# yuguangnudt/VEC_VAD

Hardware: AMD Instinct MI355X
Metric: spatio-temporal cubes/sec (train step) (higher is better)
Workload: dtype f32

## Files before the change

include/vecvad_hip.h:

```cpp
#ifndef VECVAD_HIP_H
#define VECVAD_HIP_H

#include <stddef.h>
#include <stdint.h>

#ifdef __cplusplus
extern "C" {
#endif

typedef void* vv_stream;

enum vv_status {
  VV_OK = 0,
  VV_ERR_BAD_ARG = 1,
  VV_ERR_LAUNCH = 2,
  VV_ERR_UNSUPPORTED = 3
};

enum vv_in_mode {
  VV_IN_PLAIN = 0,
  VV_IN_ACT = 1,
  VV_IN_POOL = 2,
  VV_IN_CAT = 3,
  VV_IN_CUBE = 4
};

enum vv_conv_kind {
  VV_CONV3 = 0,
  VV_CONVT_FWD = 1,
  VV_CONVT_DGRAD = 2
};

typedef struct vv_view {
  float* ptr;
  int64_t gstride;
  int32_t cstride;
  int32_t coff;
} vv_view;

#define VV_CONV_BF16 1
#define VV_CONV_SRC_BF16 2
#define VV_CONV_OUT_BF16 8
#define VV_CONV_ALLSRC_BF16 16
#define VV_CONV_RELU 32
#define VV_CONV_NO_GEMM16 64
#define VV_CONV_NO_RING 128
typedef struct vv_conv_params {
  int32_t kind;
  int32_t in_mode;
  int32_t G, B;
  int32_t H, W;
  int32_t Cin;
  int32_t CinP;
  int32_t Cout;
  vv_view src0;
  const float* a;
  const float* b;
  int64_t ab_gstride;
  vv_view src1;
  int32_t csplit;
  int32_t pad0;
  const int32_t* chmap;
  const float* w;
  int64_t w_gstride;
  const float* bias;
  int64_t bias_gstride;
  vv_view out;
  float* stats;
  const float* bn_z; int64_t bn_z_gstride;
  const float* bn_a; const float* bn_b; const float* bn_mean; const float* bn_invstd; int64_t bn_gstride;
  float* bn_partial;
  vv_view out1;
  int32_t osplit;
  int32_t pad1;
} vv_conv_params;

int vv_conv_mfma(const vv_conv_params* p, vv_stream stream);
int vv_conv_ntiles(int32_t B, int32_t H, int32_t W);
int vv_convt_dgrad_ntiles(int32_t B, int32_t H, int32_t W, int32_t flags);
int vv_conv_ntiles2(int32_t B, int32_t H, int32_t W, int32_t kind, int32_t flags);

typedef struct vv_wgrad_params {
  int32_t kind;
  int32_t in_mode;
  int32_t G, B, H, W;
  int32_t Cin, CinP, Cout;
  int32_t ksplit;
  vv_view src0; const float* a; const float* b; int64_t ab_gstride;
  vv_view src1; int32_t csplit;
  int32_t pad0;
  const int32_t* chmap;
  vv_view dy;
  float* partial;
  int64_t partial_gstride;
} vv_wgrad_params;

int vv_wgrad_mfma(const vv_wgrad_params* p, vv_stream stream);
int vv_wgrad_ntiles(int32_t kind, int32_t B, int32_t H, int32_t W);

#define VV_WGRAD_X_BF16 2
#define VV_WGRAD_DY_BF16 1
int vv_wgrad_bf16(const vv_wgrad_params* p, vv_stream stream);
int vv_wgrad_bf16_plan(int32_t kind, int32_t B, int32_t H, int32_t W, int32_t CinP, int32_t Cout, int32_t* ntiles, int32_t* nblocks,
                       int32_t* kw);

int vv_wgrad_reduce(int32_t kind, int32_t G, int32_t Cin, int32_t CinP, int32_t Cout, int32_t nslab_per_tile,
                    const float* partial, int64_t partial_gstride, float* grad, int64_t grad_gstride,
                    vv_stream stream);
typedef struct vv_reduce_entry {
  int32_t kind, Cin, Cout, NCO, nslab, block_start;
  int64_t part_off, grad_off, grad_gstride;
} vv_reduce_entry;
int vv_wgrad_reduce_grouped(const vv_reduce_entry* table_dev, int32_t nentries, int32_t total_blocks, int32_t G, const float* partial,
                            int64_t partial_gstride, float* grads, vv_stream stream);

#define VV_PACK_BF16 4
typedef struct vv_pack_entry {
  int64_t src_off;
  int64_t dst_off;
  int32_t mode, K, KP, N;
} vv_pack_entry;
int vv_pack_weights(const vv_pack_entry* table_dev, int32_t nentries, int32_t G, const float* params,
                    int64_t params_gstride, float* packed, int64_t packed_gstride, int32_t max_elems,
                    vv_stream stream);

int vv_conv_wino(const vv_conv_params* p, vv_stream stream);
int vv_wino_ntiles(int32_t B, int32_t H);
int vv_pack_wino(const vv_pack_entry* table_dev, int32_t nentries, int32_t G, const float* params, int64_t params_gstride,
                 float* packed, int64_t packed_gstride, int32_t max_kn, vv_stream stream);

int vv_conv_wino44(const vv_conv_params* p, vv_stream stream);
int vv_wino44_ntiles(int32_t B, int32_t H);
int vv_pack_wino44(const vv_pack_entry* table_dev, int32_t nentries, int32_t G, const float* params, int64_t params_gstride,
                   float* packed, int64_t packed_gstride, int32_t max_kn, vv_stream stream);

int vv_bn_finalize(int32_t G, int32_t C, int32_t ntiles, int64_t count, int32_t train, float momentum, float eps,
                   const float* stats, int64_t stats_gstride, const float* gamma, const float* beta,
                   int64_t param_gstride, float* running_mean, float* running_var, int64_t buf_gstride,
                   float* a, float* b, float* mean, float* invstd, int64_t ab_gstride, vv_stream stream);

#define VV_BNBWD_DZ_BF16 1
#define VV_BNBWD_PARTIALS_PER_CUBE 2
#define VV_BNBWD_Y_BF16 8
#define VV_BNBWD_DA_BF16 4
#define VV_BNBWD_PARTIALS_PER_TILE 16
#define VV_BNBWD_PARTIALS_PER_CTILE 32
#define VV_BNBWD_PARTIALS_PER_TTILE 128
#define VV_BNBWD_PARTIALS_PER_TILE44 64
typedef struct vv_bnbwd_params {
  int32_t G, B, H, W, C;
  int32_t flags;
  const float* y; int64_t y_gstride;
  const float* a; const float* b; const float* mean; const float* invstd; int64_t ab_gstride;
  vv_view dA;
  const float* dpool; int64_t dpool_gstride;
  float* dz; int64_t dz_gstride;
  float* partial;
} vv_bnbwd_params;
int vv_bn_bwd_reduce(const vv_bnbwd_params* p, vv_stream stream);
int vv_bn_bwd_nblk(int32_t B, int32_t H, int32_t W, int32_t C);
int vv_bn_bwd_apply(const vv_bnbwd_params* p, const float* gamma, int64_t param_gstride, float* dgamma, float* dbeta,
                    int64_t grad_gstride, float* scratch , vv_stream stream);

typedef struct vv_outconv_params {
  int32_t G, B, HW, C;
  const float* y; int64_t y_gstride; const float* a; const float* b; int64_t ab_gstride;
  const float* w; const float* bias; int64_t param_gstride;
  const int32_t* oc;
  const float* tgt0; int32_t tgt0_cstride; int32_t pad0;
  const float* tgt1; int32_t tgt1_cstride; int32_t pad1;
  const int32_t* tgt_src;
  const int32_t* tgt_coff;
  float* out4;
  float* score;
  const float* gscale;
  float* dout4;
} vv_outconv_params;
int vv_outconv_fwd(const vv_outconv_params* p, vv_stream stream);

int vv_outconv_bwd(int32_t G, int32_t B, int32_t HW, int32_t C, const float* dout4, const float* y,
                   int64_t y_gstride, const float* a, const float* b, int64_t ab_gstride, const float* w,
                   int64_t param_gstride, float* dA, int64_t dA_gstride, float* partial, const float* mean,
                   const float* invstd, float* bnpart, int32_t flags ,
                   vv_stream stream);
int vv_outconv_bwd_nblk(int32_t B, int32_t HW);
int vv_outconv_fwdbwd(const vv_outconv_params* p, float* dA, int64_t dA_gstride, float* partial, const float* mean,
                      const float* invstd, float* bnpart, int32_t flags, vv_stream stream);
int vv_outconv_bwd_reduce(int32_t G, int32_t C, int32_t nblk, const float* partial, const int32_t* oc,
                          float* dW, float* db, int64_t grad_gstride, vv_stream stream);

int vv_bias_grad(int32_t G, int64_t M, int32_t C, const float* dy, int64_t dy_gstride, int32_t cstride,
                 int32_t coff, float* scratch, float* db, int64_t grad_gstride, vv_stream stream);
int vv_bias_from_partials(int32_t G, int32_t C, int32_t ntiles, int32_t coff, int32_t n, const float* partial,
                          int64_t partial_gstride, float* db, int64_t grad_gstride, vv_stream stream);

int vv_adam(int64_t n, float* param, const float* grad, float* m, float* v, float lr, float beta1, float beta2,
            float eps, float bias_corr1, float bias_corr2_sqrt, float grad_scale, vv_stream stream);

int vv_adam_tick(int64_t* t_dev, float lr, double beta1, double beta2, float* sc_dev, vv_stream stream);
int vv_counter_add(int64_t* counters, int32_t n, int64_t inc, vv_stream stream);
int vv_adam_bucketed(int32_t G, int64_t U, int32_t nb, const int64_t* bounds, float* param, const float* grad, float* m,
                     float* v, const float* sc_dev, float beta1, float beta2, float eps, float grad_scale, vv_stream stream);

int vv_cube_gather(int32_t B, int32_t T, int32_t Tf, int32_t HW, const int64_t* idx, const uint8_t* raw,
                   const float* flow, float* x, float* xof, vv_stream stream);

int vv_pool_act(int32_t G, int32_t B, int32_t H2, int32_t W2, int32_t C, const float* y, int64_t y_gstride, const float* a,
                const float* b, int64_t ab_gstride, float* out, int64_t out_gstride, int32_t io_bf16 ,
                vv_stream stream);
int vv_cube_erase(int32_t G, int64_t npix, int32_t Cc, int32_t CP, const float* cube, const int32_t* chmap, float* out,
                  int64_t out_gstride, int32_t out_bf16, vv_stream stream);

int vv_nchw_to_nhwc(int32_t B, int32_t C, int32_t HW, const float* src, float* dst, vv_stream stream);
int vv_out4_to_nchw(int32_t B, int32_t HW, int32_t oc, const float* out4, float* dst, int32_t Ctot,
                    int32_t choff, vv_stream stream);
int vv_nchw_to_out4(int32_t B, int32_t HW, int32_t oc, const float* src, int32_t Ctot, int32_t choff,
                    float* out4, vv_stream stream);

int vv_correlation_fwd(const float* in1, const float* in2, float* out, int32_t B, int32_t C, int32_t H, int32_t W,
                       int32_t pad_size, int32_t kernel_size, int32_t max_displacement, int32_t stride1,
                       int32_t stride2, int32_t corr_type_multiply, vv_stream stream);
int vv_correlation_out_shape(int32_t C, int32_t H, int32_t W, int32_t pad_size, int32_t kernel_size,
                             int32_t max_displacement, int32_t stride1, int32_t stride2, int32_t* oC, int32_t* oH,
                             int32_t* oW);
int vv_correlation_nhwc(const float* f1, const float* f2, int32_t cstride, int32_t B, int32_t C, int32_t H, int32_t W,
                        float* out, int32_t out_cstride, int32_t out_coff, float slope, vv_stream stream);
int vv_resample2d_fwd(const float* img, const float* flow, float* out, int32_t B, int32_t C, int32_t H, int32_t W,
                      int32_t fH, int32_t fW, int32_t kernel_size, vv_stream stream);
int vv_channelnorm_fwd(const float* in, float* out, int32_t B, int32_t C, int32_t H, int32_t W, int32_t norm_deg,
                       vv_stream stream);

typedef struct vv_conv2d_params {
  int32_t kind, R, stride;
  int32_t B, H, W;
  int32_t Cin, CinP, Cout, CoutP;
  vv_view src;
  const float* w;
  const float* bias;
  float slope;
  int32_t pad0;
  vv_view out;
} vv_conv2d_params;
int vv_conv2d_mfma(const vv_conv2d_params* p, vv_stream stream);
int vv_conv2d_wino(const float* src, int32_t src_cstride, int32_t src_coff, int64_t src_elems, const float* panel, const float* bias,
                   float slope, float* out, int32_t out_cstride, int32_t out_coff, int32_t B, int32_t H, int32_t W, int32_t CinP,
// ... 70 lines not shown
```

vec_vad_amd/_lib.py:

```python
import ctypes as C
import os

import torch

HERE = os.path.dirname(os.path.abspath(__file__))
LIB_PATH = os.environ.get('VV_LIB_PATH') or os.path.join(HERE, 'csrc', 'libvecvad_hip.so')

c_i32, c_i64, c_f32, c_f64, c_vp = C.c_int32, C.c_int64, C.c_float, C.c_double, C.c_void_p

IN_PLAIN, IN_ACT, IN_POOL, IN_CAT, IN_CUBE = 0, 1, 2, 3, 4
CONV3, CONVT_FWD, CONVT_DGRAD = 0, 1, 2
CONV_BF16 = 1
CONV_SRC_BF16 = 2
PACK_BF16 = 4
BNBWD_DZ_BF16 = 1
BNBWD_PARTIALS_PER_CUBE = 2
BNBWD_DA_BF16 = 4
CONV_OUT_BF16 = 8
CONV_ALLSRC_BF16 = 16
CONV_RELU = 32
CONV_NO_GEMM16 = 64
CONV_NO_RING = 128
BNBWD_Y_BF16 = 8
BNBWD_PARTIALS_PER_TILE = 16
BNBWD_PARTIALS_PER_CTILE = 32
BNBWD_PARTIALS_PER_TILE44 = 64
BNBWD_PARTIALS_PER_TTILE = 128
WGRAD_X_BF16 = 2
WGRAD_DY_BF16 = 1


class View(C.Structure):
    _fields_ = [('ptr', c_vp), ('gstride', c_i64), ('cstride', c_i32), ('coff', c_i32)]


class ConvParams(C.Structure):
    _fields_ = [('kind', c_i32), ('in_mode', c_i32), ('G', c_i32), ('B', c_i32), ('H', c_i32), ('W', c_i32),
                ('Cin', c_i32), ('CinP', c_i32), ('Cout', c_i32),
                ('src0', View), ('a', c_vp), ('b', c_vp), ('ab_gstride', c_i64),
                ('src1', View), ('csplit', c_i32), ('pad0', c_i32), ('chmap', c_vp),
                ('w', c_vp), ('w_gstride', c_i64), ('bias', c_vp), ('bias_gstride', c_i64),
                ('out', View), ('stats', c_vp),
                ('bn_z', c_vp), ('bn_z_gstride', c_i64), ('bn_a', c_vp), ('bn_b', c_vp), ('bn_mean', c_vp), ('bn_invstd', c_vp),
                ('bn_gstride', c_i64), ('bn_partial', c_vp),
                ('out1', View), ('osplit', c_i32), ('pad1', c_i32)]


class WgradParams(C.Structure):
    _fields_ = [('kind', c_i32), ('in_mode', c_i32), ('G', c_i32), ('B', c_i32), ('H', c_i32), ('W', c_i32),
                ('Cin', c_i32), ('CinP', c_i32), ('Cout', c_i32), ('ksplit', c_i32),
                ('src0', View), ('a', c_vp), ('b', c_vp), ('ab_gstride', c_i64),
                ('src1', View), ('csplit', c_i32), ('pad0', c_i32), ('chmap', c_vp),
                ('dy', View), ('partial', c_vp), ('partial_gstride', c_i64)]


class PackEntry(C.Structure):
    _fields_ = [('src_off', c_i64), ('dst_off', c_i64), ('mode', c_i32), ('K', c_i32), ('KP', c_i32), ('N', c_i32)]


class ReduceEntry(C.Structure):
    _fields_ = [('kind', c_i32), ('Cin', c_i32), ('Cout', c_i32), ('NCO', c_i32), ('nslab', c_i32), ('block_start', c_i32),
                ('part_off', c_i64), ('grad_off', c_i64), ('grad_gstride', c_i64)]


class FoldEntry(C.Structure):
    _fields_ = [('w_off', c_i64), ('b_off', c_i64), ('g_off', c_i64), ('beta_off', c_i64), ('rm_off', c_i64), ('rv_off', c_i64),
                ('cout', c_i32), ('row', c_i32)]


class BnBwdParams(C.Structure):
    _fields_ = [('G', c_i32), ('B', c_i32), ('H', c_i32), ('W', c_i32), ('C', c_i32), ('flags', c_i32),
                ('y', c_vp), ('y_gstride', c_i64),
                ('a', c_vp), ('b', c_vp), ('mean', c_vp), ('invstd', c_vp), ('ab_gstride', c_i64),
                ('dA', View), ('dpool', c_vp), ('dpool_gstride', c_i64),
                ('dz', c_vp), ('dz_gstride', c_i64), ('partial', c_vp)]


class OutconvParams(C.Structure):
    _fields_ = [('G', c_i32), ('B', c_i32), ('HW', c_i32), ('C', c_i32),
                ('y', c_vp), ('y_gstride', c_i64), ('a', c_vp), ('b', c_vp), ('ab_gstride', c_i64),
                ('w', c_vp), ('bias', c_vp), ('param_gstride', c_i64), ('oc', c_vp),
                ('tgt0', c_vp), ('tgt0_cstride', c_i32), ('pad0', c_i32),
                ('tgt1', c_vp), ('tgt1_cstride', c_i32), ('pad1', c_i32),
                ('tgt_src', c_vp), ('tgt_coff', c_vp), ('out4', c_vp), ('score', c_vp), ('gscale', c_vp),
                ('dout4', c_vp)]


class Conv2dParams(C.Structure):
    _fields_ = [('kind', c_i32), ('R', c_i32), ('stride', c_i32), ('B', c_i32), ('H', c_i32), ('W', c_i32),
                ('Cin', c_i32), ('CinP', c_i32), ('Cout', c_i32), ('CoutP', c_i32), ('src', View), ('w', c_vp),
                ('bias', c_vp), ('slope', c_f32), ('pad0', c_i32), ('out', View)]


_SIGS = {
    'vv_conv2d_mfma': (c_i32, [C.POINTER(Conv2dParams), c_vp]),
    'vv_conv2d_wino': (c_i32, [c_vp, c_i32, c_i32, c_i64, c_vp, c_vp, c_f32, c_vp, c_i32, c_i32, c_i32, c_i32, c_i32, c_i32, c_i32, c_vp]),
    'vv_conv2d_splitk_finish': (c_i32, [c_vp, c_i32, c_i64, c_i32, c_i32, c_vp, c_f32, c_vp, c_i32, c_i32, c_vp]),
    'vv_pack_conv2d': (c_i32, [c_vp, c_vp, c_i32, c_i32, c_i32, c_i32, c_i32, c_i32, c_vp]),
    'vv_conv3x3_n2': (c_i32, [c_vp, c_i32, c_i32, c_i32, c_i32, c_i32, c_vp, c_i32, c_vp, c_f32, c_vp, c_i32, c_i32, c_vp]),
    'vv_deconv4x4_c2': (c_i32, [c_vp, c_i32, c_i32, c_i32, c_i32, c_vp, c_vp, c_f32, c_vp, c_i32, c_i32, c_vp]),
    'vv_upsample4': (c_i32, [c_vp, c_vp, c_i32, c_i32, c_i32, c_i32, c_f32, c_vp]),
    'vv_conv_mfma': (c_i32, [C.POINTER(ConvParams), c_vp]),
    'vv_conv_wino': (c_i32, [C.POINTER(ConvParams), c_vp]),
    'vv_wino_ntiles': (c_i32, [c_i32, c_i32]),
    'vv_pack_wino': (c_i32, [c_vp, c_i32, c_i32, c_vp, c_i64, c_vp, c_i64, c_i32, c_vp]),
    'vv_conv_wino44': (c_i32, [C.POINTER(ConvParams), c_vp]),
    'vv_wino44_ntiles': (c_i32, [c_i32, c_i32]),
    'vv_pack_wino44': (c_i32, [c_vp, c_i32, c_i32, c_vp, c_i64, c_vp, c_i64, c_i32, c_vp]),
    'vv_conv_ntiles': (c_i32, [c_i32, c_i32, c_i32]),
    'vv_conv_ntiles2': (c_i32, [c_i32, c_i32, c_i32, c_i32, c_i32]),
    'vv_convt_dgrad_ntiles': (c_i32, [c_i32, c_i32, c_i32, c_i32]),
    'vv_wgrad_mfma': (c_i32, [C.POINTER(WgradParams), c_vp]),
    'vv_wgrad_ntiles': (c_i32, [c_i32, c_i32, c_i32, c_i32]),
    'vv_wgrad_bf16': (c_i32, [C.POINTER(WgradParams), c_vp]),
    'vv_wgrad_bf16_plan': (c_i32, [c_i32, c_i32, c_i32, c_i32, c_i32, c_i32, C.POINTER(c_i32), C.POINTER(c_i32), C.POINTER(c_i32)]),
    'vv_wgrad_reduce': (c_i32, [c_i32, c_i32, c_i32, c_i32, c_i32, c_i32, c_vp, c_i64, c_vp, c_i64, c_vp]),
    'vv_wgrad_reduce_grouped': (c_i32, [c_vp, c_i32, c_i32, c_i32, c_vp, c_i64, c_vp, c_vp]),
    'vv_pack_weights': (c_i32, [c_vp, c_i32, c_i32, c_vp, c_i64, c_vp, c_i64, c_i32, c_vp]),
    'vv_bn_finalize': (c_i32, [c_i32, c_i32, c_i32, c_i64, c_i32, c_f32, c_f32, c_vp, c_i64, c_vp, c_vp, c_i64,
                               c_vp, c_vp, c_i64, c_vp, c_vp, c_vp, c_vp, c_i64, c_vp]),
    'vv_bn_bwd_reduce': (c_i32, [C.POINTER(BnBwdParams), c_vp]),
    'vv_bn_bwd_nblk': (c_i32, [c_i32, c_i32, c_i32, c_i32]),
    'vv_bn_bwd_apply': (c_i32, [C.POINTER(BnBwdParams), c_vp, c_i64, c_vp, c_vp, c_i64, c_vp, c_vp]),
    'vv_outconv_fwd': (c_i32, [C.POINTER(OutconvParams), c_vp]),
    'vv_outconv_bwd': (c_i32, [c_i32, c_i32, c_i32, c_i32, c_vp, c_vp, c_i64, c_vp, c_vp, c_i64, c_vp, c_i64,
                               c_vp, c_i64, c_vp, c_vp, c_vp, c_vp, c_i32, c_vp]),
    'vv_outconv_bwd_nblk': (c_i32, [c_i32, c_i32]),
    'vv_outconv_fwdbwd': (c_i32, [C.POINTER(OutconvParams), c_vp, c_i64, c_vp, c_vp, c_vp, c_vp, c_i32, c_vp]),
    'vv_outconv_bwd_reduce': (c_i32, [c_i32, c_i32, c_i32, c_vp, c_vp, c_vp, c_vp, c_i64, c_vp]),
    'vv_bias_grad': (c_i32, [c_i32, c_i64, c_i32, c_vp, c_i64, c_i32, c_i32, c_vp, c_vp, c_i64, c_vp]),
    'vv_bias_from_partials': (c_i32, [c_i32, c_i32, c_i32, c_i32, c_i32, c_vp, c_i64, c_vp, c_i64, c_vp]),
    'vv_adam': (c_i32, [c_i64, c_vp, c_vp, c_vp, c_vp, c_f32, c_f32, c_f32, c_f32, c_f32, c_f32, c_f32, c_vp]),
    'vv_adam_tick': (c_i32, [c_vp, c_f32, c_f64, c_f64, c_vp, c_vp]),
    'vv_counter_add': (c_i32, [c_vp, c_i32, c_i64, c_vp]),
    'vv_adam_bucketed': (c_i32, [c_i32, c_i64, c_i32, c_vp, c_vp, c_vp, c_vp, c_vp, c_vp, c_f32, c_f32, c_f32, c_f32, c_vp]),
    'vv_cube_gather': (c_i32, [c_i32, c_i32, c_i32, c_i32, c_vp, c_vp, c_vp, c_vp, c_vp, c_vp]),
    'vv_pool_act': (c_i32, [c_i32, c_i32, c_i32, c_i32, c_i32, c_vp, c_i64, c_vp, c_vp, c_i64, c_vp, c_i64, c_i32, c_vp]),
    'vv_cube_erase': (c_i32, [c_i32, c_i64, c_i32, c_i32, c_vp, c_vp, c_vp, c_i64, c_i32, c_vp]),
    'vv_nchw_to_nhwc': (c_i32, [c_i32, c_i32, c_i32, c_vp, c_vp, c_vp]),
    'vv_out4_to_nchw': (c_i32, [c_i32, c_i32, c_i32, c_vp, c_vp, c_i32, c_i32, c_vp]),
    'vv_nchw_to_out4': (c_i32, [c_i32, c_i32, c_i32, c_vp, c_i32, c_i32, c_vp, c_vp]),
    'vv_correlation_fwd': (c_i32, [c_vp, c_vp, c_vp, c_i32, c_i32, c_i32, c_i32, c_i32, c_i32, c_i32, c_i32, c_i32,
                                   c_i32, c_vp]),
    'vv_correlation_out_shape': (c_i32, [c_i32, c_i32, c_i32, c_i32, c_i32, c_i32, c_i32, c_i32,
                                         C.POINTER(c_i32), C.POINTER(c_i32), C.POINTER(c_i32)]),
    'vv_correlation_nhwc': (c_i32, [c_vp, c_vp, c_i32, c_i32, c_i32, c_i32, c_i32, c_vp, c_i32, c_i32, c_f32, c_vp]),
    'vv_resample2d_fwd': (c_i32, [c_vp, c_vp, c_vp, c_i32, c_i32, c_i32, c_i32, c_i32, c_i32, c_i32, c_vp]),
    'vv_channelnorm_fwd': (c_i32, [c_vp, c_vp, c_i32, c_i32, c_i32, c_i32, c_i32, c_vp]),
    'vv_fold_bn': (c_i32, [c_vp, c_i32, c_i32, c_vp, c_i64, c_vp, c_i64, c_f32, c_vp, c_i64, c_vp]),
    'vv_flownet_prep_workspace_bytes': (C.c_int64, [c_i32]),
    'vv_flownet_prep': (c_i32, [c_vp, c_i32, c_i32, c_i32, c_f32, c_vp, C.c_int64, c_vp, c_vp, c_vp, c_vp]),
    'vv_warp_pack12': (c_i32, [c_vp, c_vp, c_vp, c_i32, c_i32, c_i32, c_i32, c_i32, c_f32, c_f32, c_vp, c_vp]),
    'vv_fusion_pack11': (c_i32, [c_vp, c_vp, c_vp, c_i32, c_vp, c_i32, c_i32, c_i32, c_i32, c_f32, c_vp, c_vp]),
    'vv_crop_resize': (c_i32, [c_vp, c_i32, c_i32, c_i32, c_i32, c_i32, c_vp, c_i32, c_i32, c_i32, c_vp, c_vp]),
    'vv_frame_scores': (c_i32, [c_vp, c_vp, c_vp, c_vp, c_vp, c_vp, C.c_double, C.c_double, C.c_double, c_i32, c_vp,
                                c_vp]),
    'vv_roc_auc_counts': (c_i32, [c_vp, c_vp, c_i32, c_vp, c_vp]),
    'vv_conv2d_f16': (c_i32, [C.POINTER(Conv2dParams), c_vp]),
    'vv_pack_conv2d_f16': (c_i32, [c_vp, c_vp, c_i32, c_i32, c_i32, c_i32, c_i32, c_i32, c_vp]),
    'vv_conv2d_splitk_finish_f16': (c_i32, [c_vp, c_i32, c_i64, c_i32, c_i32, c_vp, c_f32, c_vp, c_i32, c_i32, c_vp]),
    'vv_conv3x3_n2_f16': (c_i32, [c_vp, c_i32, c_i32, c_i32, c_i32, c_i32, c_vp, c_i32, c_vp, c_f32, c_vp, c_i32, c_i32, c_vp]),
    'vv_deconv4x4_c2_f16': (c_i32, [c_vp, c_i32, c_i32, c_i32, c_i32, c_vp, c_vp, c_f32, c_vp, c_i32, c_i32, c_vp]),
    'vv_correlation_nhwc_f16': (c_i32, [c_vp, c_vp, c_i32, c_i32, c_i32, c_i32, c_i32, c_vp, c_i32, c_i32, c_f32, c_vp]),
    'vv_flownet_prep_f16': (c_i32, [c_vp, c_i32, c_i32, c_i32, c_f32, c_vp, C.c_int64, c_vp, c_vp, c_vp, c_vp]),
    'vv_warp_pack12_f16': (c_i32, [c_vp, c_vp, c_vp, c_i32, c_i32, c_i32, c_i32, c_i32, c_f32, c_f32, c_vp, c_vp]),
    'vv_fusion_pack11_f16': (c_i32, [c_vp, c_vp, c_vp, c_i32, c_vp, c_i32, c_i32, c_i32, c_i32, c_f32, c_vp, c_vp]),
    'vv_out8_to_nchw_f16': (c_i32, [c_i32, c_i32, c_i32, c_vp, c_vp, c_i32, c_i32, c_i32, c_vp]),
    'vv_version': (C.c_char_p, []),
    'vv_abi_sizeof': (c_i32, [c_i32]),
    'vv_status_string': (C.c_char_p, [c_i32]),
    'vv_device_arch_ok': (c_i32, []),
    'vv_num_cus': (c_i32, []),
}

EXPORTS = sorted(_SIGS)
ABI_STRUCTS = (View, ConvParams, WgradParams, PackEntry, ReduceEntry, FoldEntry, BnBwdParams, OutconvParams, Conv2dParams)
_lib = None


class VecVadHipError(RuntimeError):
    pass


def lib():
    global _lib
    if _lib is None:
        if not os.path.exists(LIB_PATH):
            raise VecVadHipError('libvecvad_hip.so is missing (%s). Build it with `python -m vec_vad_amd.build` '
                                 '(hipcc --offload-arch=gfx950); vec_vad_amd has no fallback path.' % LIB_PATH)
        l = C.CDLL(LIB_PATH)
        for name, (res, args) in _SIGS.items():
            f = getattr(l, name)
            f.restype = res
            f.argtypes = args
        for which, cls in enumerate(ABI_STRUCTS):
            if l.vv_abi_sizeof(which) != C.sizeof(cls):
                raise VecVadHipError('%s: sizeof(%s) is %d in the library, %d in vec_vad_amd/_lib.py -- rebuild with '
                                     '`python -m vec_vad_amd.build`' % (LIB_PATH, cls.__name__, l.vv_abi_sizeof(which), C.sizeof(cls)))
        _lib = l
    return _lib


_STATUS = {1: 'VV_ERR_BAD_ARG', 2: 'VV_ERR_LAUNCH', 3: 'VV_ERR_UNSUPPORTED'}


def check(status, what=''):
# ... 14 lines not shown
```

vec_vad_amd/bank.py:

```python
import ctypes as C
import math
import os
from collections import OrderedDict

import torch

from . import _lib as L

RAW_C, OF_C = 3, 2
HW0 = 32


def _ceil(a, b):
    return (a + b - 1) // b * b


def _pick_ksplit(groups, ntiles, ncu=256, epilogue=1.5, max_wg=1024):
    best, best_cost = 1, None
    for ks in range(1, ntiles + 1):
        if groups * ks > max_wg and ks > 1:
            break
        rounds = -(-groups * ks // ncu)
        cost = rounds * (-(-ntiles // ks) + epilogue)
        if best_cost is None or cost < best_cost - 1e-9:
# ... 681 lines not shown
                    wplan['t%d' % u] = (ks, nci * nco * ks * kw.value, kw.value)
            wmax = max(wmax, wplan['t%d' % u][1])
        woff, wtot = {}, 0
        for key, wpl in wplan.items():
            woff[key] = wtot
            wtot += wpl[1] * 9 * 1024
        ws.wpart = f(Ga, wtot)
        wpg = ws.wpart.stride(0)
        group_reduce = os.environ.get('VV_GROUP_REDUCE', '1') != '0'
        pending = []

        def flush_reduce(label, **kw_):
            ents = (L.ReduceEntry * len(pending))()
            start = 0
            for i, (key, kind, cin, cinp, cout, nslab) in enumerate(pending):
                gptr, gstride = self._g(key + '.w')
                ents[i] = L.ReduceEntry(kind, cin, cout, cout // 32, nslab, start, woff[key], (gptr - self.grads.data_ptr()) // 4, gstride)
                start += ((cinp + 31) // 32) * (cout // 32) * 36
            tab = torch.frombuffer(bytearray(bytes(ents)), dtype=torch.uint8).to(d)
            P.keep.append(tab)
            P.add(lib.vv_wgrad_reduce_grouped, (tab.data_ptr(), len(pending), start, Ga, ws.wpart.data_ptr(), wpg, self.grads.data_ptr()),
                  label, **kw_)
            del pending[:]

        y = ws.y[last.idx]
        P.add(lib.vv_outconv_bwd, (Ga, B, HWp, nf, ws.dout4.data_ptr(), y.data_ptr(), y.stride(0), self._p(ws.ab[0, last.idx]),
                                   self._p(ws.ab[1, last.idx]), abg, pbase + 4 * lay.p['o.w'][0], U, ws.gA_last.data_ptr(),
                                   ws.gA_last.stride(0), ws.ocpart.data_ptr(),
                                   self._p(ws.ab[2, last.idx]), self._p(ws.ab[3, last.idx]), ws.bnpart.data_ptr(),
                                   (1 if self.da16 else 0) | (2 if self.y16 else 0)), 'outconv_bwd')
        assert self._g('o.w')[1] == self._g('o.b')[1]
        P.add(lib.vv_outconv_bwd_reduce, (Ga, nf, B, ws.ocpart.data_ptr(), self._p(self.oc, g0), self._g('o.w')[0],
                                          self._g('o.b')[0], self._g('o.w')[1]), 'outconv_bwd_reduce')

        def dA_for(l):
            i = l.idx
            if i == last.idx:
                return L.view(ws.gA_last, nf, 0, ws.gA_last.stride(0)), None, 0
            nxt = lay.convs[i + 1] if i + 1 < len(lay.convs) else None
            cons_t = [u for u, (sidx, _, _, _) in enumerate(lay.convT) if sidx == i]
            skip_of = [m for m in lay.convs if m.mode == L.IN_CAT and m.skip == i]
            pool_of = [m for m in lay.convs if m.mode == L.IN_POOL and m.src == i]
            if cons_t:
                t = ws.DT[cons_t[0]]
                return L.view(t, t.shape[2], 0, t.stride(0)), None, 0
            if skip_of:
                m = skip_of[0]
                dp = ws.D[pool_of[0].idx] if pool_of else None
                return (dcat_views(m)[0], dp.data_ptr() if dp is not None else None,
                        dp.stride(0) if dp is not None else 0)
            m = nxt
            dn = ws.D[m.idx]
            return L.view(dn, m.cin, 0, dn.stride(0)), None, 0

        order = [l.idx for l in reversed(lay.convs)]

        def fused_producer(l):
            if not self.fuse_bn_sums or l.mode != L.IN_ACT or l.idx == 0:
                return None
            if self.wino and not self.cflag:
                pass
            elif self.y16 and self.da16 and self.dz16 and len(wplan['c%d' % l.idx]) > 2 and l.H == 32 and l.cin % 64 != 0:
                pass
            else:
                return None
            j = l.src
            if j != l.idx - 1 or j == last.idx:
                return None
            if any(sidx == j for (sidx, _, _, _) in lay.convT) or any(m.mode == L.IN_CAT and m.skip == j for m in lay.convs) \
                    or any(m.mode == L.IN_POOL and m.src == j for m in lay.convs):
                return None
            return j

        fused = {fused_producer(l) for l in lay.convs} - {None}
        fused_t = {}
        if self.fuse_bn_sums and os.environ.get('VV_FUSE_BN_SUMS_T', '1') != '0' and not self.cflag:
            for u, (sidx, _, _, _) in enumerate(lay.convT):
                others = any(m.mode == L.IN_CAT and m.skip == sidx for m in lay.convs) or any(m.mode == L.IN_POOL and m.src == sidx for m in lay.convs) \
                    or any(m.mode == L.IN_ACT and m.src == sidx for m in lay.convs)
                if not others and sidx != last.idx:
                    fused_t[u] = sidx
        fused |= set(fused_t.values())

        def dgrad_flags(i):
            dz16 = bool(self.dz16 and len(wplan['c%d' % i]) > 2)
            return (self.cflag | ((L.CONV_ALLSRC_BF16 if self.y16 else L.CONV_SRC_BF16) if dz16 else 0) |
                    (L.CONV_OUT_BF16 if self.da16 else 0))

        def conv_bwd(l):
            i = l.idx
            y = ws.y[i]
            wpl = wplan['c%d' % i]
            dz16 = bool(self.dz16 and len(wpl) > 2)
            pos = order.index(i)
            dzb = ws.dz2[pos % 2]
            reuse_wait = ('wdone%d' % order[pos - 2],) if pos >= 2 else ()
            dA, dpool, dpg = dA_for(l)
            from_outconv = i == last.idx
            from_dgrad = i in fused
            bp = L.BnBwdParams(Ga, B, l.H, l.H, l.cout,
                               (L.BNBWD_DZ_BF16 if dz16 else 0) | (L.BNBWD_PARTIALS_PER_CUBE if from_outconv else 0) |
                               ((L.BNBWD_PARTIALS_PER_TTILE if i in fused_t.values() else
                                 L.BNBWD_PARTIALS_PER_TILE44 if self._w44(B, lay.convs[i + 1], True) else L.BNBWD_PARTIALS_PER_TILE if self.wino
                                 else L.BNBWD_PARTIALS_PER_CTILE) if from_dgrad else 0) |
                               (L.BNBWD_DA_BF16 if self.da16 else 0) | (L.BNBWD_Y_BF16 if self.y16 else 0), y.data_ptr(), y.stride(0), self._p(ws.ab[0, i]), self._p(ws.ab[1, i]),
                               self._p(ws.ab[2, i]), self._p(ws.ab[3, i]), abg, dA, dpool, dpg, dzb.data_ptr(), dzb.stride(0),
                               ws.bnpart.data_ptr())
            P.keep.append(bp)
            if not (from_outconv or from_dgrad):
                P.add(lib.vv_bn_bwd_reduce, (C.byref(bp),), 'bn_bwd_reduce%d' % i, wait=reuse_wait)
            P.add(lib.vv_bn_bwd_apply, (C.byref(bp), pbase + 4 * lay.p['c%d.g' % i][0], U, self._g('c%d.g' % i)[0],
                                        self._g('c%d.beta' % i)[0], self._g('c%d.g' % i)[1], ws.bnscr.data_ptr()), 'bn_bwd_apply%d' % i,
                  record='dy%d' % i, wait=reuse_wait if (from_outconv or from_dgrad) else ())
            if i > 0:
                Dl = ws.D[i]
                w44 = self._w44(B, l, True)
                cp = L.ConvParams(L.CONV3, L.IN_PLAIN, Ga, B, l.H, l.H, l.cout, l.cout, l.cin,
                                  L.View(dzb.data_ptr(), dzb.stride(0), l.cout, 0), None, None, 0, L.NULL_VIEW, 0,
                                  dgrad_flags(i) | self.wino_flag, None,
                                  kbase + 4 * (lay.pkw44 if w44 else lay.pkw if self.wino else lay.pk)['c%d.d' % i][0], UP, None, 0,
                                  L.view(Dl, l.cin, 0, Dl.stride(0)),
                                  ws.dstats.data_ptr() if l.mode == L.IN_CAT else None)
                if l.mode == L.IN_CAT:
                    v0, v1, osplit = dcat_views(l)
                    if osplit:
                        cp.out, cp.out1, cp.osplit = v0, v1, osplit
                j = fused_producer(l)
                if j is not None:
                    yj = ws.y[j]
                    cp.bn_z, cp.bn_z_gstride = yj.data_ptr(), yj.stride(0)
                    cp.bn_a, cp.bn_b = self._p(ws.ab[0, j]), self._p(ws.ab[1, j])
                    cp.bn_mean, cp.bn_invstd = self._p(ws.ab[2, j]), self._p(ws.ab[3, j])
                    cp.bn_gstride, cp.bn_partial = abg, ws.bnpart.data_ptr()
                P.keep.append(cp)
                P.add(lib.vv_conv_wino44 if w44 else lib.vv_conv_wino if self.wino else lib.vv_conv_mfma, (C.byref(cp),), 'dgrad%d' % i,
                      record='D%d' % i, pwait=('*side',))
            mode, s0, a, b, s1, csplit, chmap = self._src_for(ws, l)
            ks, kw = wpl[0], (wpl[2] if len(wpl) > 2 else 0)
            wflag = ((L.WGRAD_DY_BF16 if dz16 else 0) | (L.WGRAD_X_BF16 if (dz16 and self.y16) else 0)) if kw else \
                (self.wgrad_flag if self.wino_wgrad else 0)
            wp = L.WgradParams(L.CONV3, mode, Ga, B, l.H, l.H, l.cin, l.cinp, l.cout, ks, s0, a, b, abg, s1, csplit,
                               wflag, chmap,
                               L.View(dzb.data_ptr(), dzb.stride(0), l.cout, 0), ws.wpart.data_ptr() + 4 * woff['c%d' % i], wpg)
            P.keep.append(wp)
            P.add(lib.vv_wgrad_bf16 if kw else lib.vv_wgrad_mfma, (C.byref(wp),), 'wgrad%d' % i, stream=1, wait=('dy%d' % i,),
                  record='wdone%d' % i, pwait=('*main',))
            if group_reduce:
                pending.append(('c%d' % i, L.CONV3, l.cin, l.cinp, l.cout, ks * max(kw, 1)))
                if i in (4, 0):
                    flush_reduce('wgrad_reduce%d' % i, stream=1)
            else:
                P.add(lib.vv_wgrad_reduce, (L.CONV3, Ga, l.cin, l.cinp, l.cout, ks * max(kw, 1), ws.wpart.data_ptr() + 4 * woff['c%d' % i], wpg)
                      + self._g('c%d.w' % i), 'wgrad_reduce%d' % i, stream=1)

        def convT_bwd(u, m):
            sidx, H, ci, co = lay.convT[u]
            skipc = lay.convs[m.skip].cout
            dy = dcat_views(m)[1]
            DT = ws.DT[u]
            cp = L.ConvParams(L.CONVT_DGRAD, L.IN_PLAIN, Ga, B, H, H, co, co, ci, dy, None, None, 0, L.NULL_VIEW, 0,
                              self.cflag | (((L.CONV_ALLSRC_BF16 if self.y16 else L.CONV_SRC_BF16) | L.CONV_OUT_BF16) if self.da16 else 0), None,
                              kbase + 4 * lay.pk['t%d.d' % u][0], UP, None, 0, L.view(DT, ci, 0, DT.stride(0)), None)
            if u in fused_t:
                yj = ws.y[sidx]
                cp.bn_z, cp.bn_z_gstride = yj.data_ptr(), yj.stride(0)
                cp.bn_a, cp.bn_b = self._p(ws.ab[0, sidx]), self._p(ws.ab[1, sidx])
                cp.bn_mean, cp.bn_invstd = self._p(ws.ab[2, sidx]), self._p(ws.ab[3, sidx])
                cp.bn_gstride, cp.bn_partial = abg, ws.bnpart.data_ptr()
            P.keep.append(cp)
            P.add(lib.vv_conv_mfma, (C.byref(cp),), 'dgradT%d' % u, pwait=('*side',))
            ntd = lib.vv_wino44_ntiles(B, m.H) if self._w44(B, m, True) else lib.vv_wino_ntiles(B, m.H) if self.wino else \
                lib.vv_conv_ntiles2(B, m.H, m.H, L.CONV3, dgrad_flags(m.idx))
            P.add(lib.vv_bias_from_partials, (Ga, m.cin, ntd, skipc, co, ws.dstats.data_ptr(), ntd * 2 * m.cin)
                  + self._g('t%d.b' % u), 'convT_bias%d' % u)
            y = ws.y[sidx]
            wpl = wplan['t%d' % u]
            ks, kw = wpl[0], (wpl[2] if len(wpl) > 2 else 0)
            wp = L.WgradParams(L.CONVT_FWD, L.IN_ACT, Ga, B, H, H, ci, ci, co, ks, L.view(y, ci, 0, y.stride(0)),
                               self._p(ws.ab[0, sidx]), self._p(ws.ab[1, sidx]), abg, L.NULL_VIEW, 0,
                               ((L.WGRAD_DY_BF16 | (L.WGRAD_X_BF16 if self.y16 else 0)) if (kw and self.da16) else 0), None, dy,
                               ws.wpart.data_ptr() + 4 * woff['t%d' % u], wpg)
            P.keep.append(wp)
            P.add(lib.vv_wgrad_bf16 if kw else lib.vv_wgrad_mfma, (C.byref(wp),), 'wgradT%d' % u, stream=1,
                  wait=('D%d' % m.idx,), pwait=('*main',))
            if group_reduce:
                pending.append(('t%d' % u, L.CONVT_FWD, ci, ci, co, ks * max(kw, 1)))
                if u == 0:
                    flush_reduce('wgradT_reduce0', stream=1, record='sideT0')
            else:
                P.add(lib.vv_wgrad_reduce, (L.CONVT_FWD, Ga, ci, ci, co, ks * max(kw, 1), ws.wpart.data_ptr() + 4 * woff['t%d' % u], wpg)
                      + self._g('t%d.w' % u), 'wgradT_reduce%d' % u, stream=1, record='sideT%d' % u)

        for l in reversed(lay.convs):
            conv_bwd(l)
            if l.mode == L.IN_CAT:
                convT_bwd(l.up, l)
        assert not pending
        return P

    def _stream(self):
        return torch.cuda.current_stream(self.device).cuda_stream

    def set_input_nchw(self, x, x_of):
        B = x.shape[0]
        ws = self.workspace(B)
        x = x.contiguous().float()
        L.check(self.lib.vv_nchw_to_nhwc(B, x.shape[1], HW0 * HW0, x.data_ptr(), ws.cube.data_ptr(), self._stream()), 'nchw_to_nhwc')
        if x_of is not None and ws.flow.numel():
            x_of = x_of.contiguous().float()
            L.check(self.lib.vv_nchw_to_nhwc(B, x_of.shape[1], HW0 * HW0, x_of.data_ptr(), ws.flow.data_ptr(), self._stream()),
                    'nchw_to_nhwc')
        return ws

    def set_input_cubes(self, raw_u8, flow, idx=None, B=None):
        B = int(idx.numel()) if idx is not None else (B if B is not None else raw_u8.shape[0])
        ws = self.workspace(B)
        L.check(self.lib.vv_cube_gather(B, self.tot_raw, self.tot_of, HW0 * HW0, idx.data_ptr() if idx is not None else None,
                                        raw_u8.data_ptr(), flow.data_ptr() if flow is not None else None, ws.cube.data_ptr(),
                                        ws.flow.data_ptr(), self._stream()), 'cube_gather')
        return ws

    def forward(self, ws, train, outputs=True):
        if not train and self.eval_fold:
            self.prepare_eval()
        plan = (ws.fwd if outputs else ws.fwdq)[bool(train)]
        plan.run(self._stream())
# ... 106 lines not shown
```

vec_vad_amd/csrc/vv_common.h:

```cpp
#pragma once
#include <hip/hip_runtime.h>
#include <stdint.h>
#include <type_traits>
#include "../../include/vecvad_hip.h"

typedef float v16f __attribute__((ext_vector_type(16)));
typedef float v4f __attribute__((ext_vector_type(4)));

#define VV_WG 256

template <int B, int E, typename F>
__device__ __forceinline__ void vv_static_for(F&& f) {
  if constexpr (B < E) {
    f(std::integral_constant<int, B>{});
    vv_static_for<B + 1, E>(f);
  }
}

#define VV_LAUNCH(...)                  \
  do {                                  \
    (void)hipGetLastError();            \
    hipLaunchKernelGGL(__VA_ARGS__);    \
  } while (0)

#define VV_HIP_STATUS(e) (VV_ERR_LAUNCH | ((int)(e) << 8))
#define VV_CHECK_LAUNCH()                                   \
  do {                                                      \
    hipError_t e__ = hipGetLastError();                     \
    if (e__ != hipSuccess) return VV_HIP_STATUS(e__);       \
  } while (0)

extern "C" int vv_num_cus(void);

int vv_conv_gemm16(const vv_conv_params* p, hipStream_t st);
inline bool vv_gemm16_flags(int kind, int flags) {
  return kind == VV_CONV3 && (flags & VV_CONV_BF16) && (flags & VV_CONV_OUT_BF16) && (flags & (VV_CONV_SRC_BF16 | VV_CONV_ALLSRC_BF16)) &&
         !(flags & VV_CONV_NO_GEMM16);
}

int vv_conv_ring16(const vv_conv_params* p, hipStream_t st);
bool vv_conv_ring16_ok(const vv_conv_params* p);

template <int N>
__device__ __forceinline__ float vv_dpp_ror(const float v) {
  return __builtin_bit_cast(float, __builtin_amdgcn_update_dpp(0, __builtin_bit_cast(int, v), 0x120 + N, 0xF, 0xF, false));
}

__device__ __forceinline__ int vv_xcd_remap(int bid, int nper) { return (bid & 7) * nper + (bid >> 3); }

__device__ __forceinline__ float4 vv_relu4(float4 v) {
  v.x = fmaxf(v.x, 0.f); v.y = fmaxf(v.y, 0.f); v.z = fmaxf(v.z, 0.f); v.w = fmaxf(v.w, 0.f);
  return v;
}
__device__ __forceinline__ float4 vv_act4(float4 v, float4 a, float4 b) {
  v.x = fmaxf(fmaf(a.x, v.x, b.x), 0.f);
  v.y = fmaxf(fmaf(a.y, v.y, b.y), 0.f);
  v.z = fmaxf(fmaf(a.z, v.z, b.z), 0.f);
  v.w = fmaxf(fmaf(a.w, v.w, b.w), 0.f);
  return v;
}
__device__ __forceinline__ float4 vv_max4(float4 p, float4 q) {
  p.x = fmaxf(p.x, q.x); p.y = fmaxf(p.y, q.y); p.z = fmaxf(p.z, q.z); p.w = fmaxf(p.w, q.w);
  return p;
}

typedef __bf16 v8bf __attribute__((ext_vector_type(8)));
typedef __bf16 v2bf __attribute__((ext_vector_type(2)));
typedef float v2f __attribute__((ext_vector_type(2)));
__device__ __forceinline__ v2f vv_pk_lo_pm_hi(const v2f x, const v2f y) {
  v2f r;
  asm("v_pk_add_f32 %0, %1, %2 op_sel:[0,1] op_sel_hi:[0,1] neg_hi:[0,1]" : "=v"(r) : "v"(x), "v"(y));
  return r;
}

template <int LPP>
__device__ __forceinline__ float vv_group_sum(float d) {
  static_assert(LPP == 8 || LPP == 16, "8 or 16 lanes per group");
  auto dpp = [](const float v, const auto CTRL) -> float {
    return __builtin_bit_cast(float, __builtin_amdgcn_update_dpp(0, __builtin_bit_cast(int, v), decltype(CTRL)::value, 0xF, 0xF, false));
  };
  d += dpp(d, std::integral_constant<int, 0xB1>{});
  d += dpp(d, std::integral_constant<int, 0x4E>{});
  d += dpp(d, std::integral_constant<int, 0x141>{});
  if constexpr (LPP == 16) d += dpp(d, std::integral_constant<int, 0x140>{});
  return d;
}

__device__ __forceinline__ uint2 vv_pack_bf16x4(float4 v) {
  const v2bf lo = __builtin_convertvector((v2f){v.x, v.y}, v2bf);
  const v2bf hi = __builtin_convertvector((v2f){v.z, v.w}, v2bf);
  uint2 o;
  o.x = __builtin_bit_cast(unsigned, lo);
  o.y = __builtin_bit_cast(unsigned, hi);
  return o;
}

__device__ __forceinline__ float4 vv_unpack_bf16x4(uint2 u) {
  return make_float4(__builtin_bit_cast(float, u.x << 16), __builtin_bit_cast(float, u.x & 0xFFFF0000u),
                     __builtin_bit_cast(float, u.y << 16), __builtin_bit_cast(float, u.y & 0xFFFF0000u));
}

struct vv_f8 { float v[8]; };
__device__ __forceinline__ vv_f8 vv_unpack_bf16x8(const uint4 u) {
  vv_f8 r;
  r.v[0] = __builtin_bit_cast(float, u.x << 16); r.v[1] = __builtin_bit_cast(float, u.x & 0xFFFF0000u);
  r.v[2] = __builtin_bit_cast(float, u.y << 16); r.v[3] = __builtin_bit_cast(float, u.y & 0xFFFF0000u);
  r.v[4] = __builtin_bit_cast(float, u.z << 16); r.v[5] = __builtin_bit_cast(float, u.z & 0xFFFF0000u);
  r.v[6] = __builtin_bit_cast(float, u.w << 16); r.v[7] = __builtin_bit_cast(float, u.w & 0xFFFF0000u);
  return r;
}
__device__ __forceinline__ uint4 vv_pack_bf16x8(const vv_f8& f) {
  const uint2 lo = vv_pack_bf16x4(make_float4(f.v[0], f.v[1], f.v[2], f.v[3]));
  const uint2 hi = vv_pack_bf16x4(make_float4(f.v[4], f.v[5], f.v[6], f.v[7]));
  return make_uint4(lo.x, lo.y, hi.x, hi.y);
}

typedef _Float16 vv_h;
typedef _Float16 v8h __attribute__((ext_vector_type(8)));
typedef _Float16 v4h __attribute__((ext_vector_type(4)));
template <typename T>
__device__ __forceinline__ float vv_rnd(const float v) {
  if constexpr (std::is_same<T, float>::value) return v;
  else return (float)(vv_h)v;
}
template <typename T>
__device__ __forceinline__ T vv_act_out(const float v, const float slope) {
  if constexpr (std::is_same<T, float>::value) {
    return v > 0.f ? v : v * slope;
  } else {
    const float r = (float)(vv_h)v;
    return (vv_h)(r > 0.f ? r : r * slope);
  }
}
template <typename T>
__device__ __forceinline__ float4 vv_ld4(const T* p) {
  if constexpr (std::is_same<T, float>::value) {
    return *reinterpret_cast<const float4*>(p);
  } else {
    const v4h h = *reinterpret_cast<const v4h*>(p);
    return make_float4((float)h.x, (float)h.y, (float)h.z, (float)h.w);
  }
}
// ... 356 lines not shown
```

vec_vad_amd/csrc/vv_conv.hip:

```cpp
#include "vv_common.h"
#ifndef VV_PD_BF
#define VV_PD_BF 1
#endif

namespace {

template <int KIND, int TH, int TW>
struct Geo {
  static constexpr int HH = KIND == VV_CONV3 ? TH + 2 : (KIND == VV_CONVT_FWD ? TH + 1 : 2 * TH + 1);
  static constexpr int HW = KIND == VV_CONV3 ? TW + 2 : (KIND == VV_CONVT_FWD ? TW + 1 : 2 * TW + 1);
  static constexpr int SP = KIND == VV_CONVT_DGRAD ? 2 : 1;
};

template <int TH, int TW, int NI, int NR, int KIND, int CK, bool BF, int S16, int MR>
__global__ void __launch_bounds__(VV_WG, (MR == 1 && BF) ? 4 : ((BF && KIND == VV_CONVT_DGRAD) ? 1 : ((NR == 1 && KIND != VV_CONVT_FWD && !(BF && NI >= 4)) ? 3 : 2)))
conv_mfma_kernel(const vv_conv_params p, const int NT, const int NN, const int total, const int nper) {
  using G_ = Geo<KIND, TH, TW>;
  constexpr int HH = G_::HH, HW = G_::HW, SP = G_::SP;
  static_assert(!BF || CK % 16 == 0, "bf16 K step = 16 channels");
  constexpr int S = BF ? CK / 2 + ((CK / 8) % 2 ? 8 : 4) : CK + 4;
  constexpr int S4 = S / 4;
  static_assert(S4 % 2 == 1, "odd float4 stride");
  static_assert(TH * TW * NI == 128 * MR, "tile pixels");
  constexpr int TN = NR * 32;
// ... 379 lines not shown
  if (H != W) return false;
  if (H == 32) { *t = {8, 32, 1}; return true; }
  if (H == 16) { *t = {16, 16, 1}; return true; }
  if (H == 8) { *t = {8, 8, 4}; return true; }
  if (H == 4) { *t = {4, 4, 16}; return true; }
  return false;
}

template <int TH, int TW, int NI, int NR, int KIND, int CK, bool BF = false, int S16 = 0, int MR = 2>
int launch(const vv_conv_params* p, hipStream_t st) {
  const int NT = ((p->B + NI - 1) / NI) * (p->H / TH) * (p->W / TW);
  const int NN = p->Cout / (NR * 32);
  const int total = p->G * NN * NT;
  const int nper = (total + 7) / 8;
  VV_LAUNCH((conv_mfma_kernel<TH, TW, NI, NR, KIND, CK, BF, S16, MR>), dim3(nper * 8), dim3(VV_WG), 0, st, *p, NT, NN,
                     total, nper);
  VV_CHECK_LAUNCH();
  return VV_OK;
}

template <int KIND, int CK, bool BF, int S16 = 0>
int dispatch(const vv_conv_params* p, hipStream_t st) {
  TileGeo t;
  if (!tile_geo(p->H, p->W, &t)) return VV_ERR_UNSUPPORTED;
  if constexpr (BF && KIND == VV_CONV3) {
    if (p->H == 16) return (p->Cout % 64) == 0 ? launch<8, 16, 1, 2, KIND, 16, BF, S16, 1>(p, st) : launch<8, 16, 1, 1, KIND, 16, BF, S16, 1>(p, st);
    if (p->H == 8) return (p->Cout % 64) == 0 ? launch<8, 8, 2, 2, KIND, 16, BF, S16, 1>(p, st) : launch<8, 8, 2, 1, KIND, 16, BF, S16, 1>(p, st);
    if (p->H == 4) return (p->Cout % 64) == 0 ? launch<4, 4, 8, 2, KIND, 16, BF, S16, 1>(p, st) : launch<4, 4, 8, 1, KIND, 16, BF, S16, 1>(p, st);
  }
  const int nt = ((p->B + t.NI - 1) / t.NI) * (p->H / t.TH) * (p->W / t.TW);
  const int64_t wide_min = (!BF && KIND == VV_CONVT_DGRAD) ? 512 : 1024;
  const bool wide = KIND != VV_CONVT_FWD && (p->Cout % 64) == 0 && (int64_t)p->G * nt * (p->Cout / 64) >= wide_min;
  constexpr int CKD = BF ? (KIND == VV_CONVT_DGRAD ? 16 : CK) : (KIND == VV_CONVT_DGRAD ? 8 : 16);
  constexpr int CK4 = BF ? 16 : 8;
  if constexpr (!BF && KIND != VV_CONV3) {
    if (p->H == 16 && KIND == VV_CONVT_DGRAD) return launch<8, 16, 1, 1, KIND, CKD, BF, S16, 1>(p, st);
    if (p->H == 8) return launch<8, 8, 2, 1, KIND, CKD, BF, S16, 1>(p, st);
    if (p->H == 4) return launch<4, 4, 8, 1, KIND, CK4, BF, S16, 1>(p, st);
  }
  if constexpr (KIND == VV_CONVT_FWD) {
    switch (p->H) {
      case 32: return launch<8, 32, 1, 1, KIND, CKD, BF, S16>(p, st);
      case 16: return launch<16, 16, 1, 1, KIND, CKD, BF, S16>(p, st);
      case 8: return launch<8, 8, 4, 1, KIND, CKD, BF, S16>(p, st);
      case 4: return launch<4, 4, 16, 1, KIND, CK4, BF, S16>(p, st);
    }
  } else {
    switch (p->H) {
      case 32: return wide ? launch<8, 32, 1, 2, KIND, CKD, BF, S16>(p, st) : launch<8, 32, 1, 1, KIND, CKD, BF, S16>(p, st);
      case 16: return wide ? launch<16, 16, 1, 2, KIND, CKD, BF, S16>(p, st) : launch<16, 16, 1, 1, KIND, CKD, BF, S16>(p, st);
      case 8: return wide ? launch<8, 8, 4, 2, KIND, CKD, BF, S16>(p, st) : launch<8, 8, 4, 1, KIND, CKD, BF, S16>(p, st);
      case 4: return wide ? launch<4, 4, 16, 2, KIND, CK4, BF, S16>(p, st) : launch<4, 4, 16, 1, KIND, CK4, BF, S16>(p, st);
    }
  }
  return VV_ERR_UNSUPPORTED;
}

}

extern "C" int vv_conv_ntiles(int32_t B, int32_t H, int32_t W) {
  TileGeo t;
  if (!tile_geo(H, W, &t)) return -1;
  return ((B + t.NI - 1) / t.NI) * (H / t.TH) * (W / t.TW);
}

extern "C" int vv_convt_dgrad_ntiles(int32_t B, int32_t H, int32_t W, int32_t flags) {
  if (H != W || (H != 16 && H != 8 && H != 4)) return -1;
  const int px = (flags & VV_CONV_BF16) ? 256 : 128;
  const int per_img = H * W;
  return per_img >= px ? B * (per_img / px) : (B + px / per_img - 1) / (px / per_img);
}

extern "C" int vv_conv_ntiles2(int32_t B, int32_t H, int32_t W, int32_t kind, int32_t flags) {
  if (vv_gemm16_flags(kind, flags)) return vv_conv_ntiles(B, H, W);
  if ((flags & VV_CONV_BF16) && kind == VV_CONV3 && H == W && H == 16) return B * 2;
  if ((flags & VV_CONV_BF16) && kind == VV_CONV3 && H == W && (H == 8 || H == 4)) return (B + (H == 8 ? 1 : 7)) / (H == 8 ? 2 : 8);
  return vv_conv_ntiles(B, H, W);
}

extern "C" int vv_conv_mfma(const vv_conv_params* p, vv_stream stream) {
  if (!p || !p->src0.ptr || !p->w || !p->out.ptr) return VV_ERR_BAD_ARG;
  if (p->G <= 0 || p->B <= 0) return VV_ERR_BAD_ARG;
  if (p->Cout % 32) return VV_ERR_UNSUPPORTED;
  hipStream_t st = (hipStream_t)stream;
  const bool bf = (p->pad0 & VV_CONV_BF16) != 0;
  if (bf && p->CinP % 16) return VV_ERR_BAD_ARG;
  if ((p->pad0 & VV_CONV_SRC_BF16) && !(bf && p->in_mode == VV_IN_PLAIN && p->kind != VV_CONVT_FWD && p->src0.coff % 2 == 0)) return VV_ERR_BAD_ARG;
  if ((p->pad0 & VV_CONV_OUT_BF16) && !bf) return VV_ERR_BAD_ARG;
  if ((p->pad0 & VV_CONV_ALLSRC_BF16) && (!bf || p->in_mode == VV_IN_POOL || p->in_mode == VV_IN_CUBE)) return VV_ERR_BAD_ARG;
  if (p->CinP % 8) return VV_ERR_BAD_ARG;
  if (p->bn_partial && !bf && p->kind == VV_CONVT_DGRAD) {
    if (p->stats || p->out1.ptr || (p->H != 16 && p->H != 8 && p->H != 4) || p->H != p->W) return VV_ERR_UNSUPPORTED;
    if (!p->bn_z || !p->bn_a || !p->bn_b || !p->bn_mean || !p->bn_invstd) return VV_ERR_BAD_ARG;
  } else if (p->bn_partial) {
    if (!(bf && (p->pad0 & VV_CONV_OUT_BF16) && (p->pad0 & VV_CONV_ALLSRC_BF16) && p->kind == VV_CONV3)) return VV_ERR_UNSUPPORTED;
    if (p->H != 32 || p->W != 32 || p->Cout % 64 == 0 || p->stats || p->out1.ptr) return VV_ERR_UNSUPPORTED;
    if (!p->bn_z || !p->bn_a || !p->bn_b || !p->bn_mean || !p->bn_invstd) return VV_ERR_BAD_ARG;
  }
  if (p->out1.ptr) {
    if (!(bf && (p->pad0 & VV_CONV_OUT_BF16) && p->kind == VV_CONV3)) return VV_ERR_UNSUPPORTED;
    if (p->osplit <= 0 || p->osplit >= p->Cout || p->osplit % 32 || p->out1.cstride != p->out.cstride ||
        p->out1.gstride != p->out.gstride || p->out1.coff % 8)
      return VV_ERR_BAD_ARG;
  }
  const int sm = !bf ? 0 : ((p->pad0 & VV_CONV_ALLSRC_BF16) ? 2 : ((p->pad0 & VV_CONV_SRC_BF16) ? 1 : 0));
  if (vv_gemm16_flags(p->kind, p->pad0) && p->H <= 16) return vv_conv_gemm16(p, st);
  if (sm == 2 && vv_conv_ring16_ok(p)) return vv_conv_ring16(p, st);
  switch (p->kind) {
    case VV_CONV3:
      if (p->CinP % 16) return VV_ERR_BAD_ARG;
      if (sm == 2 && p->bn_partial) return launch<8, 32, 1, 1, VV_CONV3, 16, true, 3>(p, st);
      if (sm == 2) return dispatch<VV_CONV3, 16, true, 2>(p, st);
      if (sm == 1) return dispatch<VV_CONV3, 16, true, 1>(p, st);
      return bf ? dispatch<VV_CONV3, 16, true>(p, st) : dispatch<VV_CONV3, 16, false>(p, st);
    case VV_CONVT_FWD:
      if (p->CinP % 16) return VV_ERR_BAD_ARG;
      if (sm == 2) return dispatch<VV_CONVT_FWD, 16, true, 2>(p, st);
      return bf ? dispatch<VV_CONVT_FWD, 16, true>(p, st) : dispatch<VV_CONVT_FWD, 16, false>(p, st);
    case VV_CONVT_DGRAD:
      if (bf && p->CinP % 16) return VV_ERR_BAD_ARG;
      if (!bf && p->bn_partial) {
        if (p->H == 16) return launch<8, 16, 1, 1, VV_CONVT_DGRAD, 8, false, 4, 1>(p, st);
        if (p->H == 8) return launch<8, 8, 2, 1, VV_CONVT_DGRAD, 8, false, 4, 1>(p, st);
        return launch<4, 4, 8, 1, VV_CONVT_DGRAD, 8, false, 4, 1>(p, st);
      }
      if (sm == 2) return dispatch<VV_CONVT_DGRAD, 8, true, 2>(p, st);
      if (sm == 1) return dispatch<VV_CONVT_DGRAD, 8, true, 1>(p, st);
      return bf ? dispatch<VV_CONVT_DGRAD, 8, true>(p, st) : dispatch<VV_CONVT_DGRAD, 8, false>(p, st);
  }
  return VV_ERR_BAD_ARG;
}
```

vec_vad_amd/csrc/vv_elem.hip:

```cpp
#include "vv_common.h"

namespace {

__global__ void __launch_bounds__(VV_WG)
pack_weights_kernel(const vv_pack_entry* __restrict__ table, const float* __restrict__ params,
                    const int64_t params_gstride, float* __restrict__ packed, const int64_t packed_gstride) {
  __shared__ float tile[8 * 32 * 9 + 8];
  const vv_pack_entry e = table[blockIdx.y];
  const int g = blockIdx.z;
  const float* src = params + (int64_t)g * params_gstride + e.src_off;
  float* dst = packed + (int64_t)g * packed_gstride + e.dst_off;
  const bool b16 = (e.mode & 4) != 0;
  const int m = e.mode & 3;
  const bool kmajor = m == 1 || m == 2;
  const bool flip = m == 1;
  const int NB = e.N >> 5, KB = e.KP >> 3;
  const int tid = threadIdx.x;
  for (int blk = blockIdx.x; blk < KB * NB; blk += gridDim.x) {
    const int kb = blk / NB, nb = blk % NB;
    const int k0 = kb * 8, n0 = nb * 32;
    __syncthreads();
    for (int i = tid; i < 8 * 32 * 9; i += VV_WG) {
      int64_t si;
      bool ok;
// ... 36 lines not shown
    a2 += (double)x2; b2 += (double)y2;
    a3 += (double)x3; b3 += (double)y3;
  }
  for (; t < n; t += VV_NP) {
    a0 += (double)st[t * step];
    b0 += (double)st[t * step + C];
  }
  s1 = (a0 + a1) + (a2 + a3);
  s2 = (b0 + b1) + (b2 + b3);
}

__global__ void __launch_bounds__(32 * VV_NP)
bn_finalize_kernel(const int C, const int ntiles, const double count, const int train, const float momentum,
                   const float eps, const float* __restrict__ stats, const int64_t stats_gstride,
                   const float* __restrict__ gamma, const float* __restrict__ beta, const int64_t param_gstride,
                   float* __restrict__ rmean, float* __restrict__ rvar, const int64_t buf_gstride,
                   float* __restrict__ a, float* __restrict__ b, float* __restrict__ mean, float* __restrict__ invstd,
                   const int64_t ab_gstride) {
  __shared__ double sh[2][VV_NP][32];
  const int g = blockIdx.y;
  const int cl = threadIdx.x & 31, part = threadIdx.x >> 5;
  const int c = blockIdx.x * 32 + cl;
  if (train) {
    double s1 = 0.0, s2 = 0.0;
    if (c < C) {
      const float* st = stats + (int64_t)g * stats_gstride + c;
      vv_sum_partials(st, ntiles, C, part, s1, s2);
    }
    sh[0][part][cl] = s1;
    sh[1][part][cl] = s2;
  }
  __syncthreads();
  if (part != 0 || c >= C) return;
  const float gm = gamma[(int64_t)g * param_gstride + c], bt = beta[(int64_t)g * param_gstride + c];
  float* rm = rmean + (int64_t)g * buf_gstride + c;
  float* rv = rvar + (int64_t)g * buf_gstride + c;
  double mu, var;
  if (train) {
    double s1 = 0.0, s2 = 0.0;
#pragma unroll
    for (int k = 0; k < VV_NP; ++k) { s1 += sh[0][k][cl]; s2 += sh[1][k][cl]; }
    mu = s1 / count;
    var = s2 / count - mu * mu;
    if (var < 0.0) var = 0.0;
    const double unb = count > 1.0 ? var * count / (count - 1.0) : var;
    *rm = (float)((1.0 - (double)momentum) * (double)*rm + (double)momentum * mu);
    *rv = (float)((1.0 - (double)momentum) * (double)*rv + (double)momentum * unb);
  } else {
    mu = (double)*rm;
    var = (double)*rv;
  }
  const double is = 1.0 / sqrt(var + (double)eps);
  const int64_t o = (int64_t)g * ab_gstride + c;
  a[o] = (float)((double)gm * is);
  b[o] = (float)((double)bt - mu * (double)gm * is);
  mean[o] = (float)mu;
  invstd[o] = (float)is;
}

template <bool POOL, int PASS>
__global__ void __launch_bounds__(VV_WG)
bn_bwd_reduce_kernel(const vv_bnbwd_params p, const int nblk, const int bp, const float* __restrict__ gamma,
                     const int64_t param_gstride, const float* __restrict__ scratch) {
  __shared__ float sh[2][VV_WG * 4];
  const int g = blockIdx.y, blk = blockIdx.x;
  const int C = p.C, Q4 = C >> 2, PL = VV_WG / Q4;
  const int q = threadIdx.x % Q4, pl = threadIdx.x / Q4;
  const int c = q * 4;
  const int64_t M = (int64_t)p.B * p.H * p.W;
  const float* __restrict__ y = p.y + (int64_t)g * p.y_gstride;
  float* __restrict__ dz = p.dz + (int64_t)g * p.dz_gstride;
  const float* __restrict__ dA = p.dA.ptr + (int64_t)g * p.dA.gstride + p.dA.coff;
  const int dcs = p.dA.cstride;
  const bool da16 = (p.flags & VV_BNBWD_DA_BF16) != 0;
  const unsigned short* __restrict__ dAh = reinterpret_cast<const unsigned short*>(p.dA.ptr + (int64_t)g * p.dA.gstride) + p.dA.coff;
  auto ldA = [&](const int64_t pix) -> float4 {
    if (da16) return vv_unpack_bf16x4(*reinterpret_cast<const uint2*>(dAh + pix * dcs + c));
    return *reinterpret_cast<const float4*>(dA + pix * dcs + c);
  };
  const int64_t abo = (int64_t)g * p.ab_gstride + c;
  const float4 a4 = *reinterpret_cast<const float4*>(p.a + abo), b4 = *reinterpret_cast<const float4*>(p.b + abo);
  const float4 m4 = *reinterpret_cast<const float4*>(p.mean + abo), i4 = *reinterpret_cast<const float4*>(p.invstd + abo);
  float4 s1 = make_float4(0, 0, 0, 0), s2 = make_float4(0, 0, 0, 0);
  float4 gk = make_float4(0, 0, 0, 0), c1 = gk, c2 = gk;
  if constexpr (PASS == 1) {
    const float4 gm = *reinterpret_cast<const float4*>(gamma + (int64_t)g * param_gstride + c);
    gk = make_float4(gm.x * i4.x, gm.y * i4.y, gm.z * i4.z, gm.w * i4.w);
    c1 = *reinterpret_cast<const float4*>(scratch + (int64_t)g * 2 * C + c);
    c2 = *reinterpret_cast<const float4*>(scratch + (int64_t)g * 2 * C + C + c);
  }

  const bool y16 = (p.flags & VV_BNBWD_Y_BF16) != 0;
  auto ldY = [&](const int64_t pix) -> float4 {
    if (y16) return vv_unpack_bf16x4(*reinterpret_cast<const uint2*>(reinterpret_cast<const unsigned short*>(y) + pix * C + c));
    return *reinterpret_cast<const float4*>(y + pix * C + c);
  };
  auto one = [&](const int64_t pix, float4 d, const float4 yv) {
    float4 z;
    z.x = fmaf(a4.x, yv.x, b4.x); z.y = fmaf(a4.y, yv.y, b4.y); z.z = fmaf(a4.z, yv.z, b4.z); z.w = fmaf(a4.w, yv.w, b4.w);
    d.x = z.x > 0.f ? d.x : 0.f; d.y = z.y > 0.f ? d.y : 0.f; d.z = z.z > 0.f ? d.z : 0.f; d.w = z.w > 0.f ? d.w : 0.f;
    const float4 xh = make_float4((yv.x - m4.x) * i4.x, (yv.y - m4.y) * i4.y, (yv.z - m4.z) * i4.z, (yv.w - m4.w) * i4.w);
    if constexpr (PASS == 0) {
      s1.x += d.x; s1.y += d.y; s1.z += d.z; s1.w += d.w;
      s2.x = fmaf(d.x, xh.x, s2.x); s2.y = fmaf(d.y, xh.y, s2.y); s2.z = fmaf(d.z, xh.z, s2.z); s2.w = fmaf(d.w, xh.w, s2.w);
    } else {
      d.x = gk.x * (d.x - c1.x - xh.x * c2.x); d.y = gk.y * (d.y - c1.y - xh.y * c2.y);
      d.z = gk.z * (d.z - c1.z - xh.z * c2.z); d.w = gk.w * (d.w - c1.w - xh.w * c2.w);
      if (p.flags & VV_BNBWD_DZ_BF16) *reinterpret_cast<uint2*>(reinterpret_cast<unsigned short*>(dz) + pix * C + c) = vv_pack_bf16x4(d);
      else *reinterpret_cast<float4*>(dz + pix * C + c) = d;
    }
  };

  const int64_t nchunks = (M + bp - 1) / bp;
  for (int64_t chunk = blk; chunk < nchunks; chunk += nblk) {
  if constexpr (!POOL) {
    for (int i = pl; i < bp; i += PL) {
      const int64_t pix = chunk * bp + i;
      if (pix < M) one(pix, ldA(pix), ldY(pix));
    }
  } else {
    const int H2 = p.H >> 1, W2 = p.W >> 1;
    const int64_t MW = M >> 2;
    const float* __restrict__ dP = p.dpool + (int64_t)g * p.dpool_gstride;
    for (int i = pl; i < (bp >> 2); i += PL) {
      const int64_t wi = chunk * (bp >> 2) + i;
      if (wi >= MW) continue;
      const int wx = (int)(wi % W2);
      const int64_t t = wi / W2;
      const int wy = (int)(t % H2);
      const int64_t img = t / H2;
      const int64_t p00 = (img * p.H + 2 * wy) * p.W + 2 * wx;
      const int64_t px[4] = {p00, p00 + 1, p00 + p.W, p00 + p.W + 1};
      float4 zz[4], yq[4];
#pragma unroll
      for (int k = 0; k < 4; ++k) {
        const float4 yv = yq[k] = ldY(px[k]);
        zz[k].x = fmaxf(fmaf(a4.x, yv.x, b4.x), 0.f); zz[k].y = fmaxf(fmaf(a4.y, yv.y, b4.y), 0.f);
        zz[k].z = fmaxf(fmaf(a4.z, yv.z, b4.z), 0.f); zz[k].w = fmaxf(fmaf(a4.w, yv.w, b4.w), 0.f);
      }
      int ix = 0, iy = 0, iz = 0, iw = 0;
      float bx = zz[0].x, by = zz[0].y, bz = zz[0].z, bw = zz[0].w;
#pragma unroll
      for (int k = 1; k < 4; ++k) {
        if (zz[k].x > bx) { bx = zz[k].x; ix = k; }
        if (zz[k].y > by) { by = zz[k].y; iy = k; }
        if (zz[k].z > bz) { bz = zz[k].z; iz = k; }
        if (zz[k].w > bw) { bw = zz[k].w; iw = k; }
      }
      const float4 dp = da16 ? vv_unpack_bf16x4(*reinterpret_cast<const uint2*>(reinterpret_cast<const unsigned short*>(dP) + wi * C + c))
                             : *reinterpret_cast<const float4*>(dP + wi * C + c);
#pragma unroll
      for (int k = 0; k < 4; ++k) {
        float4 d = ldA(px[k]);
        d.x += ix == k ? dp.x : 0.f; d.y += iy == k ? dp.y : 0.f; d.z += iz == k ? dp.z : 0.f; d.w += iw == k ? dp.w : 0.f;
        one(px[k], d, yq[k]);
      }
    }
  }
  }
  if constexpr (PASS == 1) return;
  float* r1 = sh[0];
  float* r2 = sh[1];
  *reinterpret_cast<float4*>(r1 + (pl * Q4 + q) * 4) = s1;
  *reinterpret_cast<float4*>(r2 + (pl * Q4 + q) * 4) = s2;
  __syncthreads();
  for (int ch = threadIdx.x; ch < C; ch += VV_WG) {
    float t1 = 0.f, t2 = 0.f;
    for (int k = 0; k < PL; ++k) { t1 += r1[k * C + ch]; t2 += r2[k * C + ch]; }
    float* o = p.partial + ((int64_t)(g * nblk + blk) * 2) * C + ch;
    o[0] = t1;
    o[C] = t2;
  }
}

template <bool POOL, int PASS>
__global__ void __launch_bounds__(VV_WG)
bn_bwd16_kernel(const vv_bnbwd_params p, const int nblk, const int bp, const float* __restrict__ gamma,
                const int64_t param_gstride, const float* __restrict__ scratch) {
  __shared__ float sh[2][VV_WG * 8];
  const int g = blockIdx.y, blk = blockIdx.x;
  const int C = p.C, Q8 = C >> 3, PL = VV_WG / Q8;
  const int q = threadIdx.x % Q8, pl = threadIdx.x / Q8;
  const int c = q * 8;
  const int64_t M = (int64_t)p.B * p.H * p.W;
  const unsigned short* __restrict__ yh = reinterpret_cast<const unsigned short*>(p.y + (int64_t)g * p.y_gstride);
  unsigned short* __restrict__ dzh = reinterpret_cast<unsigned short*>(p.dz + (int64_t)g * p.dz_gstride);
  const unsigned short* __restrict__ dAh = reinterpret_cast<const unsigned short*>(p.dA.ptr + (int64_t)g * p.dA.gstride) + p.dA.coff;
  const int dcs = p.dA.cstride;
  const int64_t abo = (int64_t)g * p.ab_gstride + c;
  float a[8], b[8], m[8], iv[8], s1[8], s2[8], gk[8], c1[8], c2[8];
// ... 16 lines not shown
    vv_f8 o;
#pragma unroll
    for (int j = 0; j < 8; ++j) {
      const float z = fmaf(a[j], yv.v[j], b[j]);
      const float dj = z > 0.f ? d.v[j] : 0.f;
      const float xh = (yv.v[j] - m[j]) * iv[j];
      if constexpr (PASS == 0) { s1[j] += dj; s2[j] = fmaf(dj, xh, s2[j]); }
      else o.v[j] = gk[j] * (dj - c1[j] - xh * c2[j]);
    }
    if constexpr (PASS == 1) *reinterpret_cast<uint4*>(dzh + pix * C + c) = vv_pack_bf16x8(o);
  };
  const int64_t nchunks = (M + bp - 1) / bp;
  for (int64_t chunk = blk; chunk < nchunks; chunk += nblk) {
  if constexpr (!POOL) {
    for (int i0 = pl; i0 < bp; i0 += 4 * PL) {
      uint4 qa[4], qy[4];
#pragma unroll
      for (int u = 0; u < 4; ++u) {
        const int64_t pix = chunk * bp + i0 + u * PL;
        const bool ok = i0 + u * PL < bp && pix < M;
        qa[u] = ok ? *reinterpret_cast<const uint4*>(dAh + pix * dcs + c) : make_uint4(0, 0, 0, 0);
        qy[u] = ok ? *reinterpret_cast<const uint4*>(yh + pix * C + c) : make_uint4(0, 0, 0, 0);
      }
#pragma unroll
      for (int u = 0; u < 4; ++u) {
        const int64_t pix = chunk * bp + i0 + u * PL;
        if (i0 + u * PL < bp && pix < M) one(pix, vv_unpack_bf16x8(qa[u]), vv_unpack_bf16x8(qy[u]));
      }
    }
  } else {
    const int H2 = p.H >> 1, W2 = p.W >> 1;
    const int64_t MW = M >> 2;
    const unsigned short* __restrict__ dPh = reinterpret_cast<const unsigned short*>(p.dpool + (int64_t)g * p.dpool_gstride);
    for (int i = pl; i < (bp >> 2); i += PL) {
      const int64_t wi = chunk * (bp >> 2) + i;
      if (wi >= MW) continue;
      const int wx = (int)(wi % W2);
      const int64_t t = wi / W2;
      const int wy = (int)(t % H2);
      const int64_t img = t / H2;
      const int64_t p00 = (img * p.H + 2 * wy) * p.W + 2 * wx;
      const int64_t px[4] = {p00, p00 + 1, p00 + p.W, p00 + p.W + 1};
      vv_f8 yq[4];
      int best[8];
      float bv[8];
#pragma unroll
      for (int k = 0; k < 4; ++k) {
        yq[k] = ld8(yh + px[k] * C + c);
#pragma unroll
        for (int j = 0; j < 8; ++j) {
          const float zz = fmaxf(fmaf(a[j], yq[k].v[j], b[j]), 0.f);
          if (k == 0 || zz > bv[j]) { bv[j] = zz; best[j] = k; }
        }
      }
      const vv_f8 dp = ld8(dPh + wi * C + c);
#pragma unroll
      for (int k = 0; k < 4; ++k) {
        vv_f8 d = ld8(dAh + px[k] * dcs + c);
#pragma unroll
        for (int j = 0; j < 8; ++j) d.v[j] += best[j] == k ? dp.v[j] : 0.f;
        one(px[k], d, yq[k]);
      }
    }
  }
  }
  if constexpr (PASS == 1) return;
  float* r1 = sh[0];
  float* r2 = sh[1];
#pragma unroll
  for (int j = 0; j < 8; ++j) { r1[pl * C + c + j] = s1[j]; r2[pl * C + c + j] = s2[j]; }
  __syncthreads();
  if (threadIdx.x < C) {
    float t1 = 0.f, t2 = 0.f;
    for (int k = 0; k < PL; ++k) { t1 += r1[k * C + threadIdx.x]; t2 += r2[k * C + threadIdx.x]; }
    float* o = p.partial + ((int64_t)(g * nblk + blk) * 2) * C + threadIdx.x;
    o[0] = t1;
    o[C] = t2;
  }
}

__global__ void __launch_bounds__(32 * VV_NP)
bn_bwd_sum_kernel(const int C, const int nblk, const double M, const float* __restrict__ partial,
                  float* __restrict__ dgamma, float* __restrict__ dbeta, const int64_t grad_gstride,
                  float* __restrict__ scratch) {
  __shared__ double sh[2][VV_NP][32];
  const int g = blockIdx.y;
  const int cl = threadIdx.x & 31, part = threadIdx.x >> 5;
  const int c = blockIdx.x * 32 + cl;
  double s1 = 0.0, s2 = 0.0;
  if (c < C) {
    const float* st = partial + (int64_t)g * nblk * 2 * C + c;
    vv_sum_partials(st, nblk, C, part, s1, s2);
  }
  sh[0][part][cl] = s1;
  sh[1][part][cl] = s2;
  __syncthreads();
  if (part != 0 || c >= C) return;
  s1 = 0.0; s2 = 0.0;
#pragma unroll
  for (int k = 0; k < VV_NP; ++k) { s1 += sh[0][k][cl]; s2 += sh[1][k][cl]; }
  dbeta[(int64_t)g * grad_gstride + c] = (float)s1;
  dgamma[(int64_t)g * grad_gstride + c] = (float)s2;
  scratch[(int64_t)g * 2 * C + c] = (float)(s1 / M);
  scratch[(int64_t)g * 2 * C + C + c] = (float)(s2 / M);
}

template <int CC>
__global__ void __launch_bounds__(VV_WG)
outconv_fwd_kernel(const vv_outconv_params p, const int total, const int nper) {
  constexpr int LPP = CC / 4, NPG = VV_WG / LPP;
  __shared__ float red[4];
  const int wi = vv_xcd_remap(blockIdx.x, nper);
  if (wi >= total) return;
  const int g = wi % p.G, cube = wi / p.G;
  const int tid = threadIdx.x, sub = tid % LPP, pg = tid / LPP;
  const int c = sub * 4;
  const int C = CC, oc = p.oc[g];
  const int64_t abo = (int64_t)g * p.ab_gstride + c;
  const float4 a4 = *reinterpret_cast<const float4*>(p.a + abo), b4 = *reinterpret_cast<const float4*>(p.b + abo);
  float4 wv[4];
  float bias[4];
#pragma unroll
  for (int co = 0; co < 4; ++co) {
    if (co < oc) {
      wv[co] = *reinterpret_cast<const float4*>(p.w + (int64_t)g * p.param_gstride + co * C + c);
      bias[co] = p.bias[(int64_t)g * p.param_gstride + co];
    } else {
      wv[co] = make_float4(0, 0, 0, 0);
      bias[co] = 0.f;
    }
  }
  const int tsrc = p.tgt_src[g], tco = p.tgt_coff[g];
  const float* tgt = tsrc == 0 ? p.tgt0 : p.tgt1;
  const int tcs = tsrc == 0 ? p.tgt0_cstride : p.tgt1_cstride;
  const float gs = p.gscale ? p.gscale[g] : 0.f;
  const float* __restrict__ y = p.y + (int64_t)g * p.y_gstride;
  const int64_t MB = (int64_t)p.B * p.HW;
  float sse = 0.f;
  auto ldy = [&](const int i) -> float4 {
    const int64_t pix = (int64_t)cube * p.HW + i;
    return (p.pad0 & 1) ? vv_unpack_bf16x4(*reinterpret_cast<const uint2*>(reinterpret_cast<const unsigned short*>(y) + pix * C + c))
                        : *reinterpret_cast<const float4*>(y + pix * C + c);
  };
  auto ldt = [&](const int i) -> float4 {
    float4 t = make_float4(0.f, 0.f, 0.f, 0.f);
    if (sub == 0) {
      const float* q = tgt + ((int64_t)cube * p.HW + i) * tcs + tco;
      t.x = q[0];
      if (oc > 1) t.y = q[1];
      if (oc > 2) t.z = q[2];
      if (oc > 3) t.w = q[3];
    }
    return t;
  };
  auto body = [&](const int i, const float4 yq, const float4 tq) {
    const int64_t pix = (int64_t)cube * p.HW + i;
    const float4 v = vv_act4(yq, a4, b4);
    float o[4];
#pragma unroll
    for (int co = 0; co < 4; ++co) {
      float d = v.x * wv[co].x;
      d = fmaf(v.y, wv[co].y, d); d = fmaf(v.z, wv[co].z, d); d = fmaf(v.w, wv[co].w, d);
      d = vv_group_sum<LPP>(d);
      o[co] = d + bias[co];
    }
    if (sub == 0) {
      float4 ov = make_float4(0, 0, 0, 0), dv = make_float4(0, 0, 0, 0);
      float e[4] = {0, 0, 0, 0};
      const float tv[4] = {tq.x, tq.y, tq.z, tq.w};
#pragma unroll
      for (int co = 0; co < 4; ++co)
        if (co < oc) {
          e[co] = o[co] - tv[co];
          sse = fmaf(e[co], e[co], sse);
        } else {
          o[co] = 0.f;
        }
      ov = make_float4(o[0], o[1], o[2], o[3]);
      if (p.out4) *reinterpret_cast<float4*>(p.out4 + ((int64_t)g * MB + pix) * 4) = ov;
      if (p.dout4) {
        dv = make_float4(gs * e[0], gs * e[1], gs * e[2], gs * e[3]);
        *reinterpret_cast<float4*>(p.dout4 + ((int64_t)g * MB + pix) * 4) = dv;
      }
    }
  };
  for (int i0 = pg; i0 < p.HW; i0 += 4 * NPG) {
    float4 yq4[4], tq4[4];
// ... 749 lines not shown
    if (da16) VV_OC8(32, true, true); else VV_OC8(32, true, false);
  } else if (p.C == 64) {
    if (da16) VV_OC8(64, true, true); else VV_OC8(64, true, false);
  } else return VV_ERR_UNSUPPORTED;
#undef VV_OC8
  VV_CHECK_LAUNCH();
  return VV_OK;
}

extern "C" int vv_pack_weights(const vv_pack_entry* table_dev, int32_t nentries, int32_t G, const float* params,
                               int64_t params_gstride, float* packed, int64_t packed_gstride, int32_t max_elems,
                               vv_stream stream) {
  if (!table_dev || !params || !packed || nentries <= 0) return VV_ERR_BAD_ARG;
  int bx = nblocks(max_elems, 64);
  VV_LAUNCH(pack_weights_kernel, dim3(bx, nentries, G), dim3(VV_WG), 0, (hipStream_t)stream, table_dev, params,
                     params_gstride, packed, packed_gstride);
  VV_CHECK_LAUNCH();
  return VV_OK;
}

extern "C" int vv_bn_finalize(int32_t G, int32_t C, int32_t ntiles, int64_t count, int32_t train, float momentum,
                              float eps, const float* stats, int64_t stats_gstride, const float* gamma,
                              const float* beta, int64_t param_gstride, float* running_mean, float* running_var,
                              int64_t buf_gstride, float* a, float* b, float* mean, float* invstd,
                              int64_t ab_gstride, vv_stream stream) {
  if (!gamma || !beta || !running_mean || !running_var || !a || !b || !mean || !invstd) return VV_ERR_BAD_ARG;
  if (train && !stats) return VV_ERR_BAD_ARG;
  VV_LAUNCH(bn_finalize_kernel, dim3((C + 31) / 32, G), dim3(32 * VV_NP), 0, (hipStream_t)stream, C, ntiles,
                     (double)count, train, momentum, eps, stats, stats_gstride, gamma, beta, param_gstride,
                     running_mean, running_var, buf_gstride, a, b, mean, invstd, ab_gstride);
  VV_CHECK_LAUNCH();
  return VV_OK;
}

static inline bool bn_all16(const vv_bnbwd_params* p) {
  const int all = VV_BNBWD_DZ_BF16 | VV_BNBWD_DA_BF16 | VV_BNBWD_Y_BF16;
  return (p->flags & all) == all && p->C % 8 == 0 && VV_WG % (p->C / 8) == 0 && p->dA.cstride % 8 == 0 && p->dA.coff % 8 == 0;
}

static inline int bn_bp(int C) {
  int bp = 8192 / (C > 0 ? C : 1);
  bp = bp > 256 ? 256 : (bp < 16 ? 16 : bp);
  return bp & ~3;
}
static inline int bn_bp16(int C) {
  int bp = 16384 / (C > 0 ? C : 1);
  bp = bp > 512 ? 512 : (bp < 16 ? 16 : bp);
  return bp & ~3;
}

constexpr int VV_BN_MAXBLK = 1 << 20;
extern "C" int vv_bn_bwd_nblk(int32_t B, int32_t H, int32_t W, int32_t C) {
  const int64_t M = (int64_t)B * H * W;
  const int bp = bn_bp(C);
  const int64_t n = (M + bp - 1) / bp;
  return (int)(n < VV_BN_MAXBLK ? n : VV_BN_MAXBLK);
}

static inline int bn_bp_of(const vv_bnbwd_params* p) { return bn_all16(p) ? bn_bp16(p->C) : bn_bp(p->C); }
static inline int bn_nblk_of(const vv_bnbwd_params* p) {
  const int64_t M = (int64_t)p->B * p->H * p->W;
  const int bp = bn_bp_of(p);
  const int64_t n = (M + bp - 1) / bp;
  return (int)(n < VV_BN_MAXBLK ? n : VV_BN_MAXBLK);
}

extern "C" int vv_bn_bwd_reduce(const vv_bnbwd_params* p, vv_stream stream) {
  if (!p || !p->y || !p->dA.ptr || !p->dz || !p->partial) return VV_ERR_BAD_ARG;
  if (p->C % 4 || p->C > 1024 || VV_WG % (p->C / 4)) return VV_ERR_UNSUPPORTED;
  const int nblk = bn_nblk_of(p);
  if (bn_all16(p)) {
    if (p->dpool)
      VV_LAUNCH((bn_bwd16_kernel<true, 0>), dim3(nblk, p->G), dim3(VV_WG), 0, (hipStream_t)stream, *p, nblk, bn_bp_of(p), nullptr, 0, nullptr);
    else
      VV_LAUNCH((bn_bwd16_kernel<false, 0>), dim3(nblk, p->G), dim3(VV_WG), 0, (hipStream_t)stream, *p, nblk, bn_bp_of(p), nullptr, 0, nullptr);
  } else if (p->dpool)
    VV_LAUNCH((bn_bwd_reduce_kernel<true, 0>), dim3(nblk, p->G), dim3(VV_WG), 0, (hipStream_t)stream, *p, nblk, bn_bp_of(p), nullptr, 0, nullptr);
  else
    VV_LAUNCH((bn_bwd_reduce_kernel<false, 0>), dim3(nblk, p->G), dim3(VV_WG), 0, (hipStream_t)stream, *p, nblk, bn_bp_of(p), nullptr, 0, nullptr);
  VV_CHECK_LAUNCH();
  return VV_OK;
}

extern "C" int vv_bn_bwd_apply(const vv_bnbwd_params* p, const float* gamma, int64_t param_gstride, float* dgamma,
                               float* dbeta, int64_t grad_gstride, float* scratch, vv_stream stream) {
  if (!p || !p->y || !p->dA.ptr || !p->dz || !p->partial || !gamma || !dgamma || !dbeta || !scratch) return VV_ERR_BAD_ARG;
  const int nblk = (p->flags & VV_BNBWD_PARTIALS_PER_CUBE) ? p->B
                   : (p->flags & VV_BNBWD_PARTIALS_PER_TILE) ? vv_wino_ntiles(p->B, p->H)
                   : (p->flags & VV_BNBWD_PARTIALS_PER_TILE44) ? vv_wino44_ntiles(p->B, p->H)
                   : (p->flags & VV_BNBWD_PARTIALS_PER_CTILE) ? vv_conv_ntiles(p->B, p->H, p->W)
                   : (p->flags & VV_BNBWD_PARTIALS_PER_TTILE) ? vv_convt_dgrad_ntiles(p->B, p->H, p->W, 0) : bn_nblk_of(p);
  if (nblk <= 0) return VV_ERR_BAD_ARG;
  const int nblk_apply = bn_nblk_of(p);
  const int64_t M = (int64_t)p->B * p->H * p->W;
  VV_LAUNCH(bn_bwd_sum_kernel, dim3((p->C + 31) / 32, p->G), dim3(32 * VV_NP), 0, (hipStream_t)stream, p->C, nblk, (double)M,
            p->partial, dgamma, dbeta, grad_gstride, scratch);
  VV_CHECK_LAUNCH();
  if (bn_all16(p)) {
    if (p->dpool)
      VV_LAUNCH((bn_bwd16_kernel<true, 1>), dim3(nblk_apply, p->G), dim3(VV_WG), 0, (hipStream_t)stream, *p, nblk_apply, bn_bp_of(p), gamma, param_gstride, scratch);
    else
      VV_LAUNCH((bn_bwd16_kernel<false, 1>), dim3(nblk_apply, p->G), dim3(VV_WG), 0, (hipStream_t)stream, *p, nblk_apply, bn_bp_of(p), gamma, param_gstride, scratch);
  } else if (p->dpool)
    VV_LAUNCH((bn_bwd_reduce_kernel<true, 1>), dim3(nblk_apply, p->G), dim3(VV_WG), 0, (hipStream_t)stream, *p, nblk_apply, bn_bp_of(p), gamma, param_gstride, scratch);
  else
    VV_LAUNCH((bn_bwd_reduce_kernel<false, 1>), dim3(nblk_apply, p->G), dim3(VV_WG), 0, (hipStream_t)stream, *p, nblk_apply, bn_bp_of(p), gamma, param_gstride, scratch);
  VV_CHECK_LAUNCH();
  return VV_OK;
}

extern "C" int vv_outconv_fwd(const vv_outconv_params* p, vv_stream stream) {
  if (!p || !p->y || !p->a || !p->b || !p->w || !p->bias || !p->oc || !p->tgt_src || !p->tgt_coff || !p->score || !p->tgt0)
    return VV_ERR_BAD_ARG;
  if (p->pad0 & 1) return launch_outconv8<0>(*p, nullptr, nullptr, 0, nullptr, nullptr, nullptr, nullptr, true, false, (hipStream_t)stream);
  const int total = p->B * p->G, nper = (total + 7) / 8;
  if (p->C == 32) VV_LAUNCH(outconv_fwd_kernel<32>, dim3(nper * 8), dim3(VV_WG), 0, (hipStream_t)stream, *p, total, nper);
  else if (p->C == 64) VV_LAUNCH(outconv_fwd_kernel<64>, dim3(nper * 8), dim3(VV_WG), 0, (hipStream_t)stream, *p, total, nper);
  else return VV_ERR_UNSUPPORTED;
  VV_CHECK_LAUNCH();
  return VV_OK;
}

extern "C" int vv_outconv_fwdbwd(const vv_outconv_params* p, float* dA, int64_t dA_gstride, float* partial, const float* mean,
                                 const float* invstd, float* bnpart, int32_t flags, vv_stream stream) {
  if (!p || !p->y || !p->a || !p->b || !p->w || !p->bias || !p->oc || !p->tgt_src || !p->tgt_coff || !p->score || !p->tgt0 ||
      !p->gscale || !dA || !partial)
    return VV_ERR_BAD_ARG;
  if (bnpart && (!mean || !invstd)) return VV_ERR_BAD_ARG;
  if (((flags & 2) != 0) != ((p->pad0 & 1) != 0)) return VV_ERR_BAD_ARG;
  if (flags & 2) return launch_outconv8<2>(*p, nullptr, dA, dA_gstride, partial, mean, invstd, bnpart, true, (flags & 1) != 0, (hipStream_t)stream);
  const int total = p->B * p->G, nper = (total + 7) / 8;
  if (p->C == 32) VV_LAUNCH(outconv_fwdbwd_kernel<32>, dim3(nper * 8), dim3(VV_WG), 0, (hipStream_t)stream, *p, dA, dA_gstride, partial, mean, invstd, bnpart, flags, total, nper);
  else if (p->C == 64) VV_LAUNCH(outconv_fwdbwd_kernel<64>, dim3(nper * 8), dim3(VV_WG), 0, (hipStream_t)stream, *p, dA, dA_gstride, partial, mean, invstd, bnpart, flags, total, nper);
  else return VV_ERR_UNSUPPORTED;
  VV_CHECK_LAUNCH();
  return VV_OK;
}

extern "C" int vv_outconv_bwd_nblk(int32_t B, int32_t HW) { (void)HW; return B; }

extern "C" int vv_outconv_bwd(int32_t G, int32_t B, int32_t HW, int32_t C, const float* dout4, const float* y,
                              int64_t y_gstride, const float* a, const float* b, int64_t ab_gstride, const float* w,
                              int64_t param_gstride, float* dA, int64_t dA_gstride, float* partial,
                              const float* mean, const float* invstd, float* bnpart, int32_t dA_bf16, vv_stream stream) {
  if (!dout4 || !y || !a || !b || !w || !dA || !partial) return VV_ERR_BAD_ARG;
  if (bnpart && (!mean || !invstd)) return VV_ERR_BAD_ARG;
  if (dA_bf16 & 2) {
    vv_outconv_params p = {};
    p.G = G; p.B = B; p.HW = HW; p.C = C;
    p.y = y; p.y_gstride = y_gstride; p.a = a; p.b = b; p.ab_gstride = ab_gstride;
    p.w = w; p.param_gstride = param_gstride;
    return launch_outconv8<1>(p, dout4, dA, dA_gstride, partial, mean, invstd, bnpart, true, (dA_bf16 & 1) != 0, (hipStream_t)stream);
  }
  if (C == 32)
    VV_LAUNCH(outconv_bwd_kernel<32>, dim3(B, G), dim3(VV_WG), 0, (hipStream_t)stream, B, HW, C, dout4, y, y_gstride,
              a, b, ab_gstride, w, param_gstride, dA, dA_gstride, partial, mean, invstd, bnpart, dA_bf16);
  else if (C == 64)
    VV_LAUNCH(outconv_bwd_kernel<64>, dim3(B, G), dim3(VV_WG), 0, (hipStream_t)stream, B, HW, C, dout4, y, y_gstride,
              a, b, ab_gstride, w, param_gstride, dA, dA_gstride, partial, mean, invstd, bnpart, dA_bf16);
  else return VV_ERR_UNSUPPORTED;
  VV_CHECK_LAUNCH();
  return VV_OK;
}

extern "C" int vv_outconv_bwd_reduce(int32_t G, int32_t C, int32_t nblk, const float* partial, const int32_t* oc,
                                     float* dW, float* db, int64_t grad_gstride, vv_stream stream) {
  if (!partial || !oc || !dW || !db) return VV_ERR_BAD_ARG;
  if (C == 32) VV_LAUNCH(outconv_bwd_reduce_kernel<32>, dim3(G), dim3(1024), 0, (hipStream_t)stream, C, nblk, partial, oc, dW, db, grad_gstride);
  else if (C == 64) VV_LAUNCH(outconv_bwd_reduce_kernel<64>, dim3(G), dim3(1024), 0, (hipStream_t)stream, C, nblk, partial, oc, dW, db, grad_gstride);
  else return VV_ERR_UNSUPPORTED;
  VV_CHECK_LAUNCH();
  return VV_OK;
}

extern "C" int vv_bias_grad(int32_t G, int64_t M, int32_t C, const float* dy, int64_t dy_gstride, int32_t cstride,
                            int32_t coff, float* scratch, float* db, int64_t grad_gstride, vv_stream stream) {
  if (!dy || !scratch || !db) return VV_ERR_BAD_ARG;
  if (C > VV_WG || C % 4 || VV_WG % (C / 4) || cstride % 4 || coff % 4) return VV_ERR_UNSUPPORTED;
  const int nblk = (int)((M + 1023) / 1024);
// ... 211 lines not shown
```

vec_vad_amd/csrc/vv_wgrad.hip:

```cpp
#include <cstdlib>
#include "vv_common.h"

namespace {

template <int TH, int TW, int NI, int KIND>
__global__ void __launch_bounds__(VV_WG, 1)
wgrad_mfma_kernel(const vv_wgrad_params p, const int NT, const int NCI, const int NCO, const int total, const int nper) {
  constexpr bool CT = KIND != VV_CONV3;
  constexpr int TP = TH * TW * NI;
  constexpr int PPW = TP / 4;
  constexpr int AHH = CT ? TH : TH + 2, AHW = CT ? TW : TW + 2;
  constexpr int BHH = CT ? 2 * TH + 1 : TH, BHW = CT ? 2 * TW + 1 : TW;
  constexpr int ASZ = NI * AHH * AHW * 32, BSZ = NI * BHH * BHW * 32, TSZ = ASZ + BSZ;
  constexpr bool DB = 2 * TSZ * 4 <= 160 * 1024;
  __shared__ float lds[DB ? 2 * TSZ : TSZ];
  float* lA = lds;
  float* lB = lds + ASZ;

  int w = vv_xcd_remap(blockIdx.x, nper);
  if (w >= total) return;
  const int KS = p.ksplit;
  const int ks = w % KS; w /= KS;
  const int cot = w % NCO; w /= NCO;
  const int cit = w % NCI;
// ... 90 lines not shown
        constexpr int kk = KK.value, c = kk & 1, n = c ^ 1;
        addr(tA, tB, kk + 1 < NK ? kk + 1 : 0, pa, pb);
        __builtin_amdgcn_sched_barrier(0);
        vv_static_for<0, 9>([&](auto T) {
          constexpr int t = T.value, slot = kk * 9 + t;
          mfma1(t, a[c][t], b[c]);
          if constexpr (kk + 1 < NK) {
            if constexpr (t == 0) b[n] = rd1(pa, pb);
            a[n][t] = rd(pa, pb, t);
          }
          if constexpr (slot < NPA) stA.template load_piece<slot>(sa, -1, tid);
          else if constexpr (slot < NP) stB.template load_piece<slot - NPA>(sb, 0, tid);
          else if constexpr (slot >= C0 && slot < C0 + NPA) stA.template commit_piece<slot - C0>(nA, tid);
          else if constexpr (slot >= C0 + NPA && slot < C0 + NP) stB.template commit_piece<slot - C0 - NPA>(nB, tid);
          __builtin_amdgcn_sched_barrier(0);
        });
      });
      __syncthreads();
      if (!(dbg & 2)) cur ^= 1;
    }
  } else {
  if (!(dbg & 1)) issue(ks);
  for (int pt = ks; pt < NT; pt += KS) {
    if (!(dbg & 1) && !((dbg & 2) && pt != ks)) {
      if (pt != ks) __syncthreads();
      stA.commit(lA, tid);
      stB.commit(lB, tid);
      __syncthreads();
      if (pt + KS < NT) issue(pt + KS);
    }

    float a0[9], a1[9], b0, b1;
    const float *pa, *pb;
    addr(lA, lB, 0, pa, pb);
    b0 = rd1(pa, pb);
#pragma unroll
    for (int t = 0; t < 9; ++t) a0[t] = rd(pa, pb, t);
#pragma unroll 1
    for (int kk = 0; kk < NK; kk += 2) {
      addr(lA, lB, kk + 1, pa, pb);
      __builtin_amdgcn_sched_barrier(0);
#pragma unroll
      for (int t = 0; t < 9; ++t) {
        mfma1(t, a0[t], b0);
        if (t == 0) b1 = rd1(pa, pb);
        a1[t] = rd(pa, pb, t);
        __builtin_amdgcn_sched_barrier(0);
      }
      addr(lA, lB, kk + 2 < NK ? kk + 2 : 0, pa, pb);
      __builtin_amdgcn_sched_barrier(0);
#pragma unroll
      for (int t = 0; t < 9; ++t) {
        mfma1(t, a1[t], b1);
        if (t == 0) b0 = rd1(pa, pb);
        a0[t] = rd(pa, pb, t);
        __builtin_amdgcn_sched_barrier(0);
      }
    }
  }
  }

  static_assert(TSZ >= 9 * 1024, "LDS too small for the slab");
  __syncthreads();
  for (int wv = 0; wv < 4; ++wv) {
    if (wave == wv) {
#pragma unroll
      for (int t = 0; t < 9; ++t)
#pragma unroll
        for (int i = 0; i < 16; ++i) {
          const int row = (i & 3) + 8 * (i >> 2) + 4 * half;
          float* q = lds + t * 1024 + row * 32 + l31;
          *q = wv ? *q + acc[t][i] : acc[t][i];
        }
    }
    __syncthreads();
  }
  float4* out = reinterpret_cast<float4*>(p.partial + (int64_t)g * p.partial_gstride +
                                          ((int64_t)((cit * NCO + cot) * KS + ks)) * (9 * 1024));
  const float4* l4 = reinterpret_cast<const float4*>(lds);
#pragma unroll
  for (int j = 0; j < 9; ++j) out[tid + j * VV_WG] = l4[tid + j * VV_WG];
}

template <int TH, int TW, int NI, int UH, int UNI>
__global__ void __launch_bounds__(256, 3)
wgrad_wino_kernel(const vv_wgrad_params p, const int NT, const int NCI, const int NCO, const int total, const int nper) {
  constexpr int NTH = 256, W_ = TW;
  constexpr int AHH = UH + 2, AHW = W_ + 2;
  constexpr int ASZ = UNI * AHH * AHW * 32, BSZ = UNI * UH * W_ * 32, USZ = ASZ + BSZ;
  static_assert(UNI * UH * W_ == 64, "a staged unit is 64 pixels");
  constexpr int RB = TH / UH, UPT = RB * (NI / UNI);
  constexpr int TXT = W_ / 2, TYT = UH / 2, TPI = TXT * TYT;
  constexpr int NKS = 8;
  constexpr int EXF = 4 * 3 * 16 * 64;
  constexpr int LSZ = 2 * USZ > EXF ? 2 * USZ : EXF;
  static_assert(LSZ * 4 * 3 <= 160 * 1024, "three workgroups per CU");
  constexpr int NIA = UNI * AHH * AHW * 8, NIB = 64 * 8;
  constexpr int NPA = (NIA + NTH - 1) / NTH, NPB = NIB / NTH, NP = NPA + NPB;
  constexpr int NSLOT = NKS * 4, C0 = NSLOT - NP - 1;
  static_assert(C0 >= NP + 8, "not enough MFMA slots between load issue and commit");
  constexpr unsigned OOB = 0x80000000u;
  constexpr bool ROWDYN = RB > 1;
  __shared__ float lds[LSZ];

  int w = vv_xcd_remap(blockIdx.x, nper);
  if (w >= total) return;
  const int KS = p.ksplit;
  const int ks = w % KS; w /= KS;
  const int cot = w % NCO; w /= NCO;
  const int cit = w % NCI;
  const int g = w / NCI;

  const int tid = threadIdx.x, lane = tid & 63, half = lane >> 5, l31 = lane & 31;
  const int xi = __builtin_amdgcn_readfirstlane(tid >> 6);
  const int H = p.H;
  const int tpi = H / TH;

  const VVSrc sa = vv_make_src(p, g, H, W_);
  const int q8 = tid & 7, cA = cit * 32 + q8 * 4, cB = cot * 32 + q8 * 4;
  const bool cok = cA < p.CinP;
  const bool act = (sa.mode == VV_IN_ACT) || (sa.mode == VV_IN_CAT && cA < sa.csplit);
  float4 sca = make_float4(1.f, 1.f, 1.f, 1.f), scb = make_float4(0.f, 0.f, 0.f, 0.f);
  if (act && cok) {
    sca = *reinterpret_cast<const float4*>(sa.a + cA);
    scb = *reinterpret_cast<const float4*>(sa.b + cA);
  }
  const bool second = __builtin_amdgcn_readfirstlane((int)((sa.mode == VV_IN_CAT) && cit * 32 >= sa.csplit)) != 0;
  const float* baseA = second ? sa.p1 + sa.co1 - sa.csplit : sa.p0 + sa.co0;
  const int csA = second ? sa.cs1 : sa.cs0;
  const float* baseB = p.dy.ptr + (int64_t)g * p.dy.gstride + p.dy.coff;
  const int csB = p.dy.cstride;

  unsigned voffA[NPA], voffB[NPB];
  int slotA[NPA];
  unsigned topm = 0, botm = 0;
  int imA[NPA];
#pragma unroll
  for (int k = 0; k < NPA; ++k) {
    const int it = tid + k * NTH;
    const int hp = it >> 3;
    const int hx = hp % AHW, t = hp / AHW;
    const int hy = t % AHH, im = t / AHH;
    bool ok = (NIA % NTH == 0 || it < NIA) && cok && (unsigned)(hx - 1) < (unsigned)W_;
    if (!ROWDYN) ok = ok && hy != 0 && hy != AHH - 1;
    topm |= (hy == 0) ? (1u << k) : 0u;
    botm |= (hy == AHH - 1) ? (1u << k) : 0u;
    imA[k] = im;
    voffA[k] = ok ? (unsigned)(((im * H + hy) * W_ + hx) * csA + cA) * 4u : OOB;
    slotA[k] = (NIA % NTH == 0 || it < NIA) ? hp * 32 + q8 * 4 : -1;
  }
#pragma unroll
  for (int k = 0; k < NPB; ++k) {
    const int px = (tid + k * NTH) >> 3;
    const int im = px / (UH * W_), rem = px % (UH * W_);
    voffB[k] = (unsigned)((im * H * W_ + rem) * csB + cB) * 4u;
  }

  int pt_n = ks, u_n = 0;
  float4 r[NP];
  unsigned validA = 0;
  __amdgpu_buffer_rsrc_t rsA, rsB;
  unsigned kill = 0;
  bool liveB[NPB];
  auto begin_unit = [&]() {
    const bool live = pt_n < NT;
    const int pt = live ? pt_n : ks;
    const int img0 = (pt / tpi) * NI + (u_n / RB) * UNI;
    const int uy0 = (pt % tpi) * TH + (u_n % RB) * UH;
    const int64_t oa = ((int64_t)(img0 * H + uy0 - 1) * W_ - 1) * csA;
    const int64_t ob = ((int64_t)(img0 * H + uy0) * W_) * csB;
    rsA = __builtin_amdgcn_make_buffer_rsrc(const_cast<float*>(baseA + oa), 0, 0x7FFFFFFF, 0x00020000);
    rsB = __builtin_amdgcn_make_buffer_rsrc(const_cast<float*>(baseB + ob), 0, 0x7FFFFFFF, 0x00020000);
    const bool img_ok = live && img0 < p.B;
    kill = img_ok ? 0u : 0xFFFFFFFFu;
    if (ROWDYN) {
      if (uy0 == 0) kill |= topm;
      if (uy0 + UH == H) kill |= botm;
    }
    if (UNI > 1) {
#pragma unroll
      for (int k = 0; k < NPA; ++k)
        if (img0 + imA[k] >= p.B) kill |= 1u << k;
    }
#pragma unroll
    for (int k = 0; k < NPB; ++k) {
      const int im = ((tid + k * NTH) >> 3) / (UH * W_);
      liveB[k] = live && img0 + im < p.B;
    }
    validA = 0;
    if (++u_n == UPT) { u_n = 0; pt_n += KS; }
  };
  auto load_piece = [&](auto K) {
    constexpr int k = K.value;
    if constexpr (k < NPA) {
      const bool ok = !((kill >> k) & 1u) && voffA[k] != OOB;
      validA |= ok ? (1u << k) : 0u;
      const v4f v = __builtin_amdgcn_raw_buffer_load_b128(rsA, ok ? voffA[k] : OOB, 0, 0);
      r[k] = make_float4(v.x, v.y, v.z, v.w);
    } else {
      const v4f v = __builtin_amdgcn_raw_buffer_load_b128(rsB, liveB[k - NPA] ? voffB[k - NPA] : OOB, 0, 0);
      r[k] = make_float4(v.x, v.y, v.z, v.w);
    }
  };
  auto commit_piece = [&](auto K, float* buf) {
    constexpr int k = K.value;
    if constexpr (k < NPA) {
      if (NIA % NTH == 0 || k < NPA - 1 || slotA[k] >= 0) {
        float4 v = r[k];
        if (act && ((validA >> k) & 1u)) v = vv_act4(v, sca, scb);
        *reinterpret_cast<float4*>(buf + slotA[k]) = v;
      }
    } else {
      *reinterpret_cast<float4*>(buf + ASZ + ((tid + (k - NPA) * NTH) >> 3) * 32 + q8 * 4) = r[k];
    }
  };

  const int a1 = xi == 0 ? 0 : (xi == 2 ? 2 : 1), a2 = xi == 3 ? 3 : (xi == 2 ? 1 : 2);
  const float sg = xi == 1 ? 1.f : -1.f;
  const float c0 = xi == 3 ? 0.f : 1.f, c1 = xi == 0 ? 0.f : (xi == 2 ? -1.f : 1.f);
  const int ao1 = a1 * AHW * 32, ao2 = a2 * AHW * 32;
  const int laneA = half * 64 + l31, laneB = ASZ + half * 64 + l31;
  v2f V03[2], V12[2], T[2], M12[2];
  v2f pa01, pa23, pb01, pb23, dq0, dq1;
  auto read_step = [&](const float* ub, auto J) {
    constexpr int j = J.value;
    constexpr int tt = 2 * j;
    constexpr int im = tt / TPI, rem = tt % TPI, tyl = rem / TXT, txl = rem % TXT;
    const float* pA = ub + laneA + ((im * AHH + 2 * tyl) * AHW + 2 * txl) * 32;
    const float* pB = ub + laneB + ((im * UH + 2 * tyl) * W_ + 2 * txl) * 32;
    pa01 = (v2f){pA[ao1], pA[ao1 + 32]};
    pa23 = (v2f){pA[ao1 + 64], pA[ao1 + 96]};
    pb01 = (v2f){pA[ao2], pA[ao2 + 32]};
    pb23 = (v2f){pA[ao2 + 64], pA[ao2 + 96]};
    dq0 = (v2f){pB[0], pB[32]};
    dq1 = (v2f){pB[W_ * 32], pB[W_ * 32 + 32]};
  };
  auto xform_step = [&](auto SET) {
    constexpr int st = SET.value;
    const v2f r01 = __builtin_elementwise_fma((v2f){sg, sg}, pb01, pa01);
    const v2f r23 = __builtin_elementwise_fma((v2f){sg, sg}, pb23, pa23);
    V03[st] = r01 - r23;
    V12[st] = vv_pk_lo_pm_hi(r23, r01);
    const v2f t = __builtin_elementwise_fma((v2f){c1, c1}, dq1, c0 * dq0);
    T[st] = t;
    M12[st] = vv_pk_lo_pm_hi(t, t);
  };

  v16f acc[4];
#pragma unroll
  for (int n = 0; n < 4; ++n)
#pragma unroll
    for (int i = 0; i < 16; ++i) acc[n][i] = 0.f;

  begin_unit();
  vv_static_for<0, NP>([&](auto K) { load_piece(K); });
  vv_static_for<0, NP>([&](auto K) { commit_piece(K, lds); });
  __syncthreads();
  const int nunits = ((NT - ks + KS - 1) / KS) * UPT;
  int cur = 0;
  for (int un = 0; un < nunits; ++un) {
    const float* ub = lds + cur * USZ;
    float* nb = lds + (cur ^ 1) * USZ;
    begin_unit();
    read_step(ub, std::integral_constant<int, 0>{});
    xform_step(std::integral_constant<int, 0>{});
    __builtin_amdgcn_sched_barrier(0);
    vv_static_for<0, NKS>([&](auto JJ) {
      constexpr int j = JJ.value, st = j & 1;
      constexpr bool more = j + 1 < NKS;
      vv_static_for<0, 4>([&](auto NN) {
        constexpr int nu = NN.value, slot = j * 4 + nu;
        const float va = nu == 0 ? V03[st].x : (nu == 1 ? V12[st].x : (nu == 2 ? V12[st].y : V03[st].y));
        const float mb = nu == 0 ? T[st].x : (nu == 1 ? M12[st].x : (nu == 2 ? M12[st].y : T[st].y));
        acc[nu] = __builtin_amdgcn_mfma_f32_32x32x2f32(va, mb, acc[nu], 0, 0, 0);
        if constexpr (more && nu == 0) read_step(ub, std::integral_constant<int, j + 1>{});
        if constexpr (more && nu == 2) xform_step(std::integral_constant<int, st ^ 1>{});
        if constexpr (slot < NP) load_piece(std::integral_constant<int, slot>{});
        else if constexpr (slot >= C0 && slot < C0 + NP) commit_piece(std::integral_constant<int, slot - C0>{}, nb);
        __builtin_amdgcn_sched_barrier(0);
      });
    });
    __syncthreads();
    cur ^= 1;
  }

  const float sx = xi == 3 ? -1.f : 1.f;
  float* ex = lds + lane;
#pragma unroll
  for (int i = 0; i < 16; ++i) {
    const float u0 = acc[0][i], u1 = acc[1][i], u2 = acc[2][i], u3 = -acc[3][i];
    const float hs = 0.5f * (u1 + u2);
    ex[((xi * 3 + 0) * 16 + i) * 64] = sx * (u0 + hs);
    ex[((xi * 3 + 1) * 16 + i) * 64] = sx * (0.5f * (u1 - u2));
    ex[((xi * 3 + 2) * 16 + i) * 64] = sx * (u3 + hs);
  }
  __syncthreads();
  float* out = p.partial + (int64_t)g * p.partial_gstride + ((int64_t)((cit * NCO + cot) * KS + ks)) * (9 * 1024);
#pragma unroll
  for (int j = 0; j < 4; ++j) {
    const int i = xi * 4 + j;
    const int row = j + 8 * xi + 4 * half;
#pragma unroll
    for (int b = 0; b < 3; ++b) {
      const float d0 = ex[((0 * 3 + b) * 16 + i) * 64], d1 = ex[((1 * 3 + b) * 16 + i) * 64];
      const float d2 = ex[((2 * 3 + b) * 16 + i) * 64], d3 = ex[((3 * 3 + b) * 16 + i) * 64];
      const float hs = 0.5f * (d1 + d2);
      out[(0 * 3 + b) * 1024 + row * 32 + l31] = d0 + hs;
      out[(1 * 3 + b) * 1024 + row * 32 + l31] = 0.5f * (d1 - d2);
      out[(2 * 3 + b) * 1024 + row * 32 + l31] = d3 + hs;
    }
  }
}

__global__ void __launch_bounds__(VV_WG)
wgrad_reduce_kernel(const int kind, const int Cin, const int Cout, const int NCO, const int nslab,
                    const float* __restrict__ partial, const int64_t partial_gstride, float* __restrict__ grad,
                    const int64_t grad_gstride) {
  const int quarter = blockIdx.x & 3;
  const int tap = (blockIdx.x >> 2) % 9;
  const int tile = (blockIdx.x >> 2) / 9;
  const int g = blockIdx.y;
  const int cit = tile / NCO, cot = tile % NCO;
  const int e = quarter * VV_WG + threadIdx.x;
  const float* src = partial + (int64_t)g * partial_gstride + (int64_t)tile * nslab * (9 * 1024) + tap * 1024 + e;
  float s0 = 0.f, s1 = 0.f, s2 = 0.f, s3 = 0.f;
  int k = 0;
  for (; k + 4 <= nslab; k += 4) {
    s0 += src[(int64_t)(k + 0) * (9 * 1024)];
    s1 += src[(int64_t)(k + 1) * (9 * 1024)];
    s2 += src[(int64_t)(k + 2) * (9 * 1024)];
    s3 += src[(int64_t)(k + 3) * (9 * 1024)];
  }
  for (; k < nslab; ++k) s0 += src[(int64_t)k * (9 * 1024)];
  const float s = (s0 + s1) + (s2 + s3);
  float* dst = grad + (int64_t)g * grad_gstride;
  const int ci = cit * 32 + (e >> 5), co = cot * 32 + (e & 31);
  if (ci < Cin && co < Cout) {
    if (kind == VV_CONV3) dst[((int64_t)co * Cin + ci) * 9 + tap] = s;
    else dst[((int64_t)ci * Cout + co) * 9 + tap] = s;
  }
}

__global__ void __launch_bounds__(VV_WG)
wgrad_reduce_grouped_kernel(const vv_reduce_entry* __restrict__ table, const int n, const float* __restrict__ partial,
                            const int64_t partial_gstride, float* __restrict__ grads) {
  int e = 0;
  for (int i = 1; i < n; ++i) e = (int)blockIdx.x >= table[i].block_start ? i : e;
  const vv_reduce_entry t = table[e];
  const int bx = blockIdx.x - t.block_start;
  const int quarter = bx & 3;
  const int tap = (bx >> 2) % 9;
  const int tile = (bx >> 2) / 9;
  const int g = blockIdx.y;
  const int cit = tile / t.NCO, cot = tile % t.NCO;
  const int el = quarter * VV_WG + threadIdx.x;
  const float* src = partial + (int64_t)g * partial_gstride + t.part_off + (int64_t)tile * t.nslab * (9 * 1024) + tap * 1024 + el;
  float s0 = 0.f, s1 = 0.f, s2 = 0.f, s3 = 0.f;
  int k = 0;
  for (; k + 4 <= t.nslab; k += 4) {
    s0 += src[(int64_t)(k + 0) * (9 * 1024)];
    s1 += src[(int64_t)(k + 1) * (9 * 1024)];
    s2 += src[(int64_t)(k + 2) * (9 * 1024)];
    s3 += src[(int64_t)(k + 3) * (9 * 1024)];
  }
  for (; k < t.nslab; ++k) s0 += src[(int64_t)k * (9 * 1024)];
  const float s = (s0 + s1) + (s2 + s3);
  float* dst = grads + t.grad_off + (int64_t)g * t.grad_gstride;
  const int ci = cit * 32 + (el >> 5), co = cot * 32 + (el & 31);
  if (ci < t.Cin && co < t.Cout) {
    if (t.kind == VV_CONV3) dst[((int64_t)co * t.Cin + ci) * 9 + tap] = s;
    else dst[((int64_t)ci * t.Cout + co) * 9 + tap] = s;
  }
}

inline bool wgradT_tile64() {
  static const int v = [] { const char* e = getenv("VV_WGRADT_TILE64"); return (e && e[0] == '0') ? 0 : 1; }();
  return v != 0;
}

struct WGeo { int TH, TW, NI; };
inline bool wgeo(int kind, int H, int W, WGeo* t) {
  if (H != W) return false;
  if (kind == VV_CONV3) {
    if (H == 32) { *t = {8, 32, 1}; return true; }
    if (H == 16) { *t = {16, 16, 1}; return true; }
    if (H == 8) { *t = {8, 8, 2}; return true; }
    if (H == 4) { *t = {4, 4, 8}; return true; }
  } else if (wgradT_tile64()) {
    if (H == 16) { *t = {4, 16, 1}; return true; }
    if (H == 8) { *t = {4, 8, 2}; return true; }
    if (H == 4) { *t = {4, 4, 4}; return true; }
  } else {
    if (H == 16) { *t = {8, 16, 1}; return true; }
    if (H == 8) { *t = {8, 8, 2}; return true; }
    if (H == 4) { *t = {4, 4, 8}; return true; }
  }
  return false;
}

template <int TH, int TW, int NI, int UH, int UNI>
int launch_ww(const vv_wgrad_params* p, hipStream_t st) {
  if (p->W != TW) return VV_ERR_UNSUPPORTED;
  const int NT = ((p->B + NI - 1) / NI) * (p->H / TH) * (p->W / TW);
  const int NCI = (p->CinP + 31) / 32, NCO = p->Cout / 32;
  const int total = p->G * NCI * NCO * p->ksplit;
  const int nper = (total + 7) / 8;
  VV_LAUNCH((wgrad_wino_kernel<TH, TW, NI, UH, UNI>), dim3(nper * 8), dim3(256), 0, st, *p, NT, NCI, NCO, total, nper);
  VV_CHECK_LAUNCH();
  return VV_OK;
}

template <int TH, int TW, int NI, int KIND>
int launch_w(const vv_wgrad_params* p, hipStream_t st) {
  const int NT = ((p->B + NI - 1) / NI) * (p->H / TH) * (p->W / TW);
  const int NCI = (p->CinP + 31) / 32, NCO = p->Cout / 32;
  const int total = p->G * NCI * NCO * p->ksplit;
  const int nper = (total + 7) / 8;
  VV_LAUNCH((wgrad_mfma_kernel<TH, TW, NI, KIND>), dim3(nper * 8), dim3(VV_WG), 0, st, *p, NT, NCI, NCO, total,
                     nper);
  VV_CHECK_LAUNCH();
  return VV_OK;
}

}

extern "C" int vv_wgrad_ntiles(int32_t kind, int32_t B, int32_t H, int32_t W) {
  WGeo t;
  if (!wgeo(kind, H, W, &t)) return -1;
  return ((B + t.NI - 1) / t.NI) * (H / t.TH) * (W / t.TW);
}

extern "C" int vv_wgrad_mfma(const vv_wgrad_params* p, vv_stream stream) {
  if (!p || !p->src0.ptr || !p->dy.ptr || !p->partial) return VV_ERR_BAD_ARG;
  if (p->Cout % 32 || p->ksplit < 1) return VV_ERR_BAD_ARG;
  if (p->kind == VV_CONV3 && (p->in_mode == VV_IN_POOL || p->in_mode == VV_IN_CUBE))
    return VV_ERR_UNSUPPORTED;
  hipStream_t st = (hipStream_t)stream;
  if (p->kind == VV_CONV3 && (p->pad0 & 256)) {
    switch (p->H) {
      case 32: return launch_ww<8, 32, 1, 2, 1>(p, st);
      case 16: return launch_ww<16, 16, 1, 4, 1>(p, st);
      case 8: return launch_ww<8, 8, 2, 8, 1>(p, st);
      case 4: return launch_ww<4, 4, 8, 4, 4>(p, st);
    }
    return VV_ERR_UNSUPPORTED;
  }
  if (p->kind == VV_CONV3) {
    switch (p->H) {
      case 32: return launch_w<8, 32, 1, VV_CONV3>(p, st);
      case 16: return launch_w<16, 16, 1, VV_CONV3>(p, st);
      case 8: return launch_w<8, 8, 2, VV_CONV3>(p, st);
      case 4: return launch_w<4, 4, 8, VV_CONV3>(p, st);
    }
  } else if (wgradT_tile64()) {
    switch (p->H) {
      case 16: return launch_w<4, 16, 1, VV_CONVT_FWD>(p, st);
      case 8: return launch_w<4, 8, 2, VV_CONVT_FWD>(p, st);
      case 4: return launch_w<4, 4, 4, VV_CONVT_FWD>(p, st);
    }
  } else {
    switch (p->H) {
      case 16: return launch_w<8, 16, 1, VV_CONVT_FWD>(p, st);
      case 8: return launch_w<8, 8, 2, VV_CONVT_FWD>(p, st);
      case 4: return launch_w<4, 4, 8, VV_CONVT_FWD>(p, st);
    }
  }
  return VV_ERR_UNSUPPORTED;
}

extern "C" int vv_wgrad_reduce(int32_t kind, int32_t G, int32_t Cin, int32_t CinP, int32_t Cout,
                               int32_t nslab_per_tile, const float* partial, int64_t partial_gstride, float* grad,
                               int64_t grad_gstride, vv_stream stream) {
  if (!partial || !grad) return VV_ERR_BAD_ARG;
  const int NCI = (CinP + 31) / 32, NCO = Cout / 32;
  VV_LAUNCH(wgrad_reduce_kernel, dim3(NCI * NCO * 9 * 4, G), dim3(VV_WG), 0, (hipStream_t)stream, kind, Cin, Cout,
                     NCO, nslab_per_tile, partial, partial_gstride, grad, grad_gstride);
  VV_CHECK_LAUNCH();
  return VV_OK;
}

extern "C" int vv_wgrad_reduce_grouped(const vv_reduce_entry* table_dev, int32_t nentries, int32_t total_blocks, int32_t G,
                                       const float* partial, int64_t partial_gstride, float* grads, vv_stream stream) {
  if (!table_dev || !partial || !grads || nentries <= 0 || total_blocks <= 0) return VV_ERR_BAD_ARG;
  VV_LAUNCH(wgrad_reduce_grouped_kernel, dim3(total_blocks, G), dim3(VV_WG), 0, (hipStream_t)stream, table_dev, nentries, partial,
            partial_gstride, grads);
  VV_CHECK_LAUNCH();
  return VV_OK;
}
```

vec_vad_amd/csrc/vv_wgrad_bf16.hip:

```cpp
#include "vv_common.h"

namespace {

typedef unsigned v4u __attribute__((ext_vector_type(4)));
typedef short v4s __attribute__((ext_vector_type(4)));
typedef __attribute__((address_space(3))) char* vv_lds_t;

__device__ __forceinline__ vv_lds_t vv_lds_ptr(float* p) { return (vv_lds_t)p; }

__device__ __forceinline__ v8bf vv_tr8(const vv_lds_t p, const int o0, const int o1) {
  const v4s lo = __builtin_amdgcn_ds_read_tr16_b64_v4i16((__attribute__((address_space(3))) v4s*)(p + o0));
  const v4s hi = __builtin_amdgcn_ds_read_tr16_b64_v4i16((__attribute__((address_space(3))) v4s*)(p + o1));
  typedef short v8s __attribute__((ext_vector_type(8)));
  return __builtin_bit_cast(v8bf, __builtin_shufflevector(lo, hi, 0, 1, 2, 3, 4, 5, 6, 7));
}

template <int TH, int TW, int NI, int CB, int OB, bool DY16, bool A16>
__global__ void __launch_bounds__(VV_WG, 1)
wgrad_bf16_kernel(const vv_wgrad_params p, const int NT, const int NCI, const int NCO, const int total, const int nper) {
  constexpr int KW = 4 / (CB * OB);
  constexpr int RL = KW == 4 ? 4 : 8;
  constexpr int NSEG = KW == 1 ? 2 : 1;
  constexpr int AHH = TH + 2, AHW = TW + 2;
  constexpr int S = 16;
// ... 705 lines not shown
  const int NCI = (p->CinP + 31) / 32, NCO = p->Cout / 32;
  if (p->ksplit > NT) return VV_ERR_BAD_ARG;
  const int total = p->G * (NCI / CB) * (NCO / OB) * p->ksplit;
  const int nper = (total + 7) / 8;
  VV_LAUNCH((wgrad_ring_kernel<TH, TW, NI, CB, OB, NBUF>), dim3(nper * 8), dim3(2 * VV_WG), 0, st, *p, NT, NCI, NCO, total, nper);
  VV_CHECK_LAUNCH();
  return VV_OK;
}

inline void ring_block_shape(int H, int NCI, int NCO, int* cbk, int* obk) {
  (void)H;
  *cbk = NCI % 2 == 0 ? 2 : 1;
  *obk = NCO % 2 == 0 ? 2 : 1;
}

inline bool ring_planned(int kind, int flags, int H, int W, int CinP, int Cout, RGeo* r, int* cbk, int* obk) {
  const int both = VV_WGRAD_X_BF16 | VV_WGRAD_DY_BF16;
  if (kind != VV_CONV3 || (flags & both) != both || Cout % 32 || CinP <= 0 || CinP % 8) return false;
  const int NCI = (CinP + 31) / 32, NCO = Cout / 32;
  ring_block_shape(H, NCI, NCO, cbk, obk);
  return rgeo(H, W, *cbk == 1 && *obk == 1, r);
}

inline bool ring_ok(const vv_wgrad_params* p) {
  const int both = VV_WGRAD_X_BF16 | VV_WGRAD_DY_BF16;
  if (p->kind != VV_CONV3 || (p->pad0 & both) != both || p->H != p->W || p->H < 8) return false;
  if (p->in_mode != VV_IN_PLAIN && p->in_mode != VV_IN_ACT && p->in_mode != VV_IN_CAT) return false;
  if (p->src0.cstride % 8 || p->src0.coff % 8 || p->dy.cstride % 8 || p->dy.coff % 8 || p->CinP % 8) return false;
  if (p->in_mode == VV_IN_CAT && (p->csplit % 32 || p->src1.cstride % 8 || p->src1.coff % 8)) return false;
  return true;
}

int dispatch_r(const vv_wgrad_params* p, hipStream_t st) {
  const int NCI = (p->CinP + 31) / 32, NCO = p->Cout / 32;
  int c, o;
  const int H = p->H == p->W ? p->H : 0;
  ring_block_shape(H, NCI, NCO, &c, &o);
#define VV_RING(H_, TH1, NI1, TH2, NI2, TW_)                                                   \
  if (H == H_) {                                                                                \
    if (c == 1 && o == 1) return launch_r<TH1, TW_, NI1, 1, 1, (H_ == 8 ? 3 : 4)>(p, st);        \
    if (c == 2 && o == 1) return launch_r<TH2, TW_, NI2, 2, 1, 3>(p, st);                       \
    if (c == 1 && o == 2) return launch_r<TH2, TW_, NI2, 1, 2, 3>(p, st);                       \
    return launch_r<TH2, TW_, NI2, 2, 2, 3>(p, st);                                             \
  }
  VV_RING(32, 8, 1, 4, 1, 32)
  VV_RING(16, 16, 1, 8, 1, 16)
  VV_RING(8, 8, 4, 8, 2, 8)
#undef VV_RING
  return VV_ERR_UNSUPPORTED;
}

}

extern "C" int vv_wgrad_bf16_plan(int32_t kind, int32_t B, int32_t H, int32_t W, int32_t CinP, int32_t Cout, int32_t* ntiles,
                                  int32_t* nblocks, int32_t* kw) {
  const int flags = kind >> 8;
  kind &= 0xff;
  {
    RGeo r;
    int cbk, obk;
    if (ring_planned(kind, flags, H, W, CinP, Cout, &r, &cbk, &obk)) {
      const int NCI = (CinP + 31) / 32, NCO = Cout / 32;
      if (ntiles) *ntiles = ((B + r.NI - 1) / r.NI) * (H / r.TH);
      if (nblocks) *nblocks = (NCI / cbk) * (NCO / obk);
      if (kw) *kw = 1;
      return 1;
    }
  }
  BGeo t;
  if (!bgeo(kind, H, W, &t) || Cout % 32 || CinP <= 0) return 0;
  const int NCI = (CinP + 31) / 32, NCO = Cout / 32;
  int cbk, obk;
  block_shape(kind, t.TW, NCI, NCO, &cbk, &obk);
  if (ntiles) *ntiles = ((B + t.NI - 1) / t.NI) * (H / t.TH) * (W / t.TW);
  if (nblocks) *nblocks = (NCI / cbk) * (NCO / obk);
  if (kw) *kw = 1;
  return 1;
}

extern "C" int vv_wgrad_bf16(const vv_wgrad_params* p, vv_stream stream) {
  if (!p || !p->src0.ptr || !p->dy.ptr || !p->partial) return VV_ERR_BAD_ARG;
  if (p->Cout % 32 || p->ksplit < 1) return VV_ERR_BAD_ARG;
  if (p->in_mode == VV_IN_POOL || p->in_mode == VV_IN_CUBE) return VV_ERR_UNSUPPORTED;
  hipStream_t st = (hipStream_t)stream;
  if ((p->pad0 & VV_WGRAD_DY_BF16) && p->dy.coff % 2) return VV_ERR_BAD_ARG;
  if ((p->pad0 & VV_WGRAD_X_BF16) && !(p->pad0 & VV_WGRAD_DY_BF16)) return VV_ERR_UNSUPPORTED;
  if (ring_ok(p)) return dispatch_r(p, st);
  {
    RGeo r;
    int cbk, obk;
    if (ring_planned(p->kind, p->pad0, p->H, p->W, p->CinP, p->Cout, &r, &cbk, &obk))
      return VV_ERR_BAD_ARG;
  }
  if (p->kind != VV_CONV3) {
    switch (p->H == p->W ? p->H : 0) {
      case 16: return dispatch_t<8, 16, 1>(p, st);
      case 8: return dispatch_t<8, 8, 2>(p, st);
      case 4: return dispatch_t<4, 4, 8>(p, st);
    }
    return VV_ERR_UNSUPPORTED;
  }
  switch (p->H == p->W ? p->H : 0) {
    case 32: return dispatch_b<8, 32, 1>(p, st);
    case 16: return dispatch_b<16, 16, 1>(p, st);
    case 8: return dispatch_b<8, 8, 4>(p, st);
    case 4: return dispatch_b<4, 4, 16>(p, st);
  }
  return VV_ERR_UNSUPPORTED;
}
```

vec_vad_amd/csrc/vv_wino.hip:

```cpp
#include <cstdlib>
#include <type_traits>
#include "vv_common.h"
#ifndef VV_RING_D
#define VV_RING_D 4
#endif
#ifndef VV_RING_MIN
#define VV_RING_MIN (4 * 512)
#endif
namespace {

constexpr int WN = 256;
constexpr int WT = 32;
constexpr int SB_MASK = 0x386;

__device__ __forceinline__ void vv_lds_barrier() {
  asm volatile("s_waitcnt lgkmcnt(0)" ::: "memory");
  __builtin_amdgcn_s_barrier();
  asm volatile("" ::: "memory");
}

template <int H_>
struct WGeo {
  static constexpr int TPI = H_ / 2;
  static constexpr int TP = TPI * TPI;
  static constexpr int TPW = TP < WT ? TP : WT;
  static constexpr int NI = WT / TPW;
  static constexpr int PARTS = TP / TPW;
  static constexpr int TROWS = TPW / TPI;
  static constexpr int HH = 2 * TROWS + 2, HW = H_ + 2;
};

template <int H_, int NB>
__global__ void __launch_bounds__(WN, NB == 2 ? 2 : 3)
wino_conv_kernel(const vv_conv_params p, const int NT, const int NN, const int total, const int nper) {
  using G_ = WGeo<H_>;
  constexpr int TPI = G_::TPI, TPW = G_::TPW, NI = G_::NI, PARTS = G_::PARTS, HH = G_::HH, HW = G_::HW, HWH = HW / 2;
  constexpr int CK = 8, S = CK + 4, S4 = S / 4, Q = CK / 4;
  constexpr int A4 = NI * HH * HW * S4;
  constexpr int NITEMS = NI * HH * HW * Q;
  constexpr int NIT = (NITEMS + WN - 1) / WN;
  constexpr int EX4 = 4 * 16 * 64 / 2;
  constexpr int L4 = A4 > EX4 ? A4 : EX4;
  static_assert(WN % Q == 0, "one channel group per thread");
  __shared__ float4 lds4[L4 + 64];
  float* lds = reinterpret_cast<float*>(lds4);
  const v4f* ldsA = reinterpret_cast<const v4f*>(lds4);

  int w = vv_xcd_remap(blockIdx.x, nper);
  if (w >= total) return;
  const int nn = w % NN; w /= NN;
  const int pt = w % NT;
  const int g = w / NT;

  const int tid = threadIdx.x, lane = tid & 63, half = lane >> 5, l31 = lane & 31;
  const int xi = __builtin_amdgcn_readfirstlane(tid >> 6);
  const int img0 = (pt / PARTS) * NI, part = pt % PARTS;
  const int y0 = part * (2 * G_::TROWS) - 1;
  const VVSrc s = vv_make_src(p, g, H_, H_);
  const int Cout = p.Cout, CinP = p.CinP, KQ = CinP >> 3;
  const int co0 = nn * 32 * NB;
  const float* __restrict__ wg = p.w + (int64_t)g * p.w_gstride;

  float4 r[NIT];
  int slot[NIT];
  unsigned valid = 0;
  unsigned voff[NIT];
  int pixv[NIT];
  const int tile = (img0 * H_ + y0) * H_ - 1;
  const int q4 = (tid % Q) * 4;
#pragma unroll
  for (int k = 0; k < NIT; ++k) {
    const int it = tid + k * WN;
    const int q = it % Q, hp = it / Q;
    const int hx = hp % HW, t = hp / HW;
    const int hy = t % HH, im = t / HH;
    const bool inr = NITEMS % WN == 0 || it < NITEMS;
    const int y = y0 + hy;
    const bool ok = inr && (unsigned)(hx - 1) < (unsigned)H_ && (unsigned)y < (unsigned)H_ && (img0 + im) < s.B;
    valid |= ok ? (1u << k) : 0u;
    pixv[k] = (im * H_ + hy) * H_ + hx;
    slot[k] = inr ? ((im * HH + hy) * HW + (hx & 1) * HWH + (hx >> 1)) * S4 + q : -1;
  }
  const __amdgpu_buffer_rsrc_t rsW = __builtin_amdgcn_make_buffer_rsrc(const_cast<float*>(wg), 0, 0x7FFFFFFF, 0x00020000);
  const unsigned bvo = (unsigned)(half * Cout + co0 + l31) * 16u;
  const int bnu = KQ * 2 * Cout * 16;
  const int bxi = xi * 4 * bnu;
  float4 sa, sb;
  bool act = false;
  __amdgpu_buffer_rsrc_t rs;
  int cur_second = -1, soff0 = 0;
  auto set_source = [&](const bool second) {
    const float* base = second ? s.p1 + s.co1 : s.p0 + s.co0;
    const int cs = second ? s.cs1 : s.cs0;
    rs = __builtin_amdgcn_make_buffer_rsrc(const_cast<float*>(base), 0, 0x7FFFFFFF, 0x00020000);
    soff0 = second ? -s.csplit * 4 : 0;
#pragma unroll
    for (int k = 0; k < NIT; ++k)
      voff[k] = ((valid >> k) & 1u) ? (unsigned)((tile + pixv[k]) * cs + q4) * 4u : 0x80000000u;
    cur_second = second ? 1 : 0;
  };
  auto issue = [&](const int c0) {
    const int c = c0 + q4;
    act = (s.mode == VV_IN_ACT) || (s.mode == VV_IN_CAT && c < s.csplit);
    if (act) {
      sa = *reinterpret_cast<const float4*>(s.a + c);
      sb = *reinterpret_cast<const float4*>(s.b + c);
    }
    const int second = __builtin_amdgcn_readfirstlane((int)((s.mode == VV_IN_CAT) && c0 >= s.csplit));
    if (second != cur_second) set_source(second != 0);
#pragma unroll
    for (int k = 0; k < NIT; ++k) {
      const v4f v = __builtin_amdgcn_raw_buffer_load_b128(rs, voff[k], c0 * 4 + soff0, 0);
      r[k] = make_float4(v.x, v.y, v.z, v.w);
    }
  };
  auto commit = [&]() {
#pragma unroll
    for (int k = 0; k < NIT; ++k)
      if (NITEMS % WN == 0 || k < NIT - 1 || slot[k] >= 0) {
        float4 v = r[k];
        if (act && ((valid >> k) & 1u)) v = vv_act4(v, sa, sb);
        lds4[slot[k]] = v;
      }
  };
  auto load_u = [&](const int c0, const int n, const int nb) -> v4f {
    return __builtin_amdgcn_raw_buffer_load_b128(rsW, bvo + nb * 512u, bxi + n * bnu + (c0 >> 3) * 2 * Cout * 16, 0);
  };

  const int tim = l31 / TPW, trem = l31 % TPW;
  const int tyl = trem / TPI, tx = trem % TPI;
  const int pbase = ((tim * HH + 2 * tyl) * HW + tx) * S4 + half;
  auto patch = [&](const int a, const int b) -> v4f {
    return ldsA[pbase + (a * HW + (b & 1) * HWH + (b >> 1)) * S4];
  };
  const int a1 = xi == 0 ? 0 : (xi == 2 ? 2 : 1), a2 = xi == 3 ? 3 : (xi == 2 ? 1 : 2);
  const float sg = xi == 1 ? 1.f : -1.f;

  v16f acc[NB][4];
  v4f u[NB][4];
  const int klast = CinP - CK;
  auto compute = [&](const int c0, const auto first, const auto more) {
    const int kn = c0 + CK;
    const int knext = kn < klast ? kn : klast;
    if constexpr (decltype(more)::value) issue(kn);
    v4f R[4];
#pragma unroll
    for (int b = 0; b < 4; ++b) {
      const v4f d1 = patch(a1, b), d2 = patch(a2, b);
      R[b] = d1 + sg * d2;
    }
    v4f V[4];
    V[0] = R[0] - R[2];
    V[1] = R[1] + R[2];
    V[2] = R[2] - R[1];
    V[3] = R[1] - R[3];
    __builtin_amdgcn_sched_barrier(SB_MASK);
#pragma unroll
    for (int n = 0; n < 4; ++n) {
#pragma unroll
      for (int nb = 0; nb < NB; ++nb) {
        if constexpr (decltype(first)::value) {
          const v16f z = {0.f, 0.f, 0.f, 0.f, 0.f, 0.f, 0.f, 0.f, 0.f, 0.f, 0.f, 0.f, 0.f, 0.f, 0.f, 0.f};
          acc[nb][n] = __builtin_amdgcn_mfma_f32_32x32x2f32(V[n].x, u[nb][n].x, z, 0, 0, 0);
        } else {
          acc[nb][n] = __builtin_amdgcn_mfma_f32_32x32x2f32(V[n].x, u[nb][n].x, acc[nb][n], 0, 0, 0);
        }
        acc[nb][n] = __builtin_amdgcn_mfma_f32_32x32x2f32(V[n].y, u[nb][n].y, acc[nb][n], 0, 0, 0);
        acc[nb][n] = __builtin_amdgcn_mfma_f32_32x32x2f32(V[n].z, u[nb][n].z, acc[nb][n], 0, 0, 0);
        acc[nb][n] = __builtin_amdgcn_mfma_f32_32x32x2f32(V[n].w, u[nb][n].w, acc[nb][n], 0, 0, 0);
        u[nb][n] = load_u(knext, n, nb);
        __builtin_amdgcn_sched_barrier(SB_MASK);
      }
    }
  };

  issue(0);
#pragma unroll
  for (int n = 0; n < 4; ++n)
#pragma unroll
    for (int nb = 0; nb < NB; ++nb) u[nb][n] = load_u(0, n, nb);
  commit();
  __syncthreads();
  const std::true_type yes{};
  const std::false_type no{};
  if (CK >= CinP) {
    compute(0, yes, no);
  } else {
    compute(0, yes, yes);
    int c0 = CK;
    for (; c0 + CK < CinP; c0 += CK) {
      __syncthreads();
      commit();
      __syncthreads();
      compute(c0, no, yes);
    }
    __syncthreads();
    commit();
    __syncthreads();
    compute(c0, no, no);
  }

#pragma unroll
  for (int nb = 0; nb < NB; ++nb) {
    const int cob = co0 + nb * 32;
// ... 416 lines not shown
    flush_stats();
  }
  asm volatile("s_waitcnt vmcnt(0)" ::: "memory");
}

__global__ void __launch_bounds__(VV_WG)
wino_pack_kernel(const vv_pack_entry* __restrict__ table, const float* __restrict__ params, const int64_t params_gstride,
                 float* __restrict__ packed, const int64_t packed_gstride) {
  __shared__ float ex[16][256];
  const vv_pack_entry e = table[blockIdx.y];
  const int g = blockIdx.z;
  const float* src = params + (int64_t)g * params_gstride + e.src_off;
  float* dst = packed + (int64_t)g * packed_gstride + e.dst_off;
  const int KQ = e.KP >> 3, NB = e.N >> 5;
  const int t = threadIdx.x, kl = t & 7, nl = t >> 3;
  for (int blk = blockIdx.x; blk < KQ * NB; blk += gridDim.x) {
    const int kq = blk / NB, nb = blk % NB;
    const int k = kq * 8 + kl, n = nb * 32 + nl;
    float gk[3][3];
#pragma unroll
    for (int a = 0; a < 3; ++a)
#pragma unroll
      for (int b = 0; b < 3; ++b) {
        float v = 0.f;
        if (k < e.K) v = e.mode == 0 ? src[((int64_t)n * e.K + k) * 9 + a * 3 + b]
                                     : src[((int64_t)k * e.N + n) * 9 + (2 - a) * 3 + (2 - b)];
        gk[a][b] = v;
      }
    float r[4][3];
#pragma unroll
    for (int b = 0; b < 3; ++b) {
      r[0][b] = gk[0][b];
      r[1][b] = 0.5f * (gk[0][b] + gk[1][b] + gk[2][b]);
      r[2][b] = 0.5f * (gk[0][b] - gk[1][b] + gk[2][b]);
      r[3][b] = gk[2][b];
    }
    const int slot = (kl >> 2) * 128 + nl * 4 + (kl & 3);
    __syncthreads();
#pragma unroll
    for (int xi = 0; xi < 4; ++xi) {
      ex[xi * 4 + 0][slot] = r[xi][0];
      ex[xi * 4 + 1][slot] = 0.5f * (r[xi][0] + r[xi][1] + r[xi][2]);
      ex[xi * 4 + 2][slot] = 0.5f * (r[xi][0] - r[xi][1] + r[xi][2]);
      ex[xi * 4 + 3][slot] = r[xi][2];
    }
    __syncthreads();
    const int hf = t >> 7, rem = t & 127;
#pragma unroll
    for (int xn = 0; xn < 16; ++xn)
      dst[((((int64_t)xn * KQ + kq) * 2 + hf) * e.N + nb * 32) * 4 + rem] = ex[xn][t];
  }
}

template <int KQ>
int launch_wino_ring(const vv_conv_params* p, hipStream_t st) {
  const int NT = p->B * 8;
  const int NN = p->Cout / 32;
  const int total = p->G * NN * NT;
  const int slots = 2 * vv_num_cus();
  const int ipw = (total + slots - 1) / slots;
  const int nwg = (total + ipw - 1) / ipw;
  if (p->bn_partial)
    VV_LAUNCH((wino_ring_kernel<KQ, true, false>), dim3(nwg), dim3(WN), 0, st, *p, NT, NN, total, ipw);
  else if (p->pad0 & VV_CONV_RELU)
    VV_LAUNCH((wino_ring_kernel<KQ, false, true>), dim3(nwg), dim3(WN), 0, st, *p, NT, NN, total, ipw);
  else
    VV_LAUNCH((wino_ring_kernel<KQ, false, false>), dim3(nwg), dim3(WN), 0, st, *p, NT, NN, total, ipw);
  VV_CHECK_LAUNCH();
  return VV_OK;
}

inline bool vv_wino_ring_ok(const vv_conv_params* p) {
  if (p->H != 32 || (p->CinP != 16 && p->CinP != 32) || (p->pad0 & VV_CONV_NO_RING)) return false;
  if (p->in_mode != VV_IN_PLAIN && p->in_mode != VV_IN_ACT) return false;
  if (p->bn_partial && (p->pad0 & VV_CONV_RELU)) return false;
  return (int64_t)p->G * (p->Cout / 32) * p->B * 8 >= VV_RING_MIN;
}

template <int H_>
int launch_wino(const vv_conv_params* p, hipStream_t st) {
  using G_ = WGeo<H_>;
  const int NT = ((p->B + G_::NI - 1) / G_::NI) * G_::PARTS;
  static const bool nb1 = [] { const char* e = getenv("VV_WINO_NB"); return e && e[0] == '1'; }();
  bool two = !nb1 && p->Cout % 64 == 0;
  if (two) {
    const int64_t wgs = (int64_t)p->G * (p->Cout / 64) * NT;
    const int64_t rounds = (wgs + 511) / 512;
    two = wgs >= 1024 && wgs * 10 >= rounds * 512 * 9;
  }
  const int NN = p->Cout / (two ? 64 : 32);
  const int total = p->G * NN * NT;
  const int nper = (total + 7) / 8;
  if (two)
    VV_LAUNCH((wino_conv_kernel<H_, 2>), dim3(nper * 8), dim3(WN), 0, st, *p, NT, NN, total, nper);
  else
    VV_LAUNCH((wino_conv_kernel<H_, 1>), dim3(nper * 8), dim3(WN), 0, st, *p, NT, NN, total, nper);
  VV_CHECK_LAUNCH();
  return VV_OK;
}

}

extern "C" int vv_wino_ntiles(int32_t B, int32_t H) {
  switch (H) {
    case 32: return ((B + WGeo<32>::NI - 1) / WGeo<32>::NI) * WGeo<32>::PARTS;
    case 16: return ((B + WGeo<16>::NI - 1) / WGeo<16>::NI) * WGeo<16>::PARTS;
    case 8: return ((B + WGeo<8>::NI - 1) / WGeo<8>::NI) * WGeo<8>::PARTS;
    case 4: return ((B + WGeo<4>::NI - 1) / WGeo<4>::NI) * WGeo<4>::PARTS;
  }
  return -1;
}

extern "C" int vv_conv_wino(const vv_conv_params* p, vv_stream stream) {
  if (!p || !p->src0.ptr || !p->w || !p->out.ptr) return VV_ERR_BAD_ARG;
  if (p->G <= 0 || p->B <= 0 || p->kind != VV_CONV3 || p->H != p->W) return VV_ERR_BAD_ARG;
  if (p->Cout % 32 || p->CinP % 8) return VV_ERR_UNSUPPORTED;
  if (p->out1.ptr) return VV_ERR_UNSUPPORTED;
  if (p->bn_partial && (p->stats || !p->bn_z || !p->bn_a || !p->bn_b || !p->bn_mean || !p->bn_invstd)) return VV_ERR_BAD_ARG;
  {
    const int64_t px = (int64_t)p->B * p->H * p->W * 4;
    const int64_t cs = p->out.cstride > p->Cout ? p->out.cstride : p->Cout;
    if (px * cs >= (1ll << 31)) return VV_ERR_UNSUPPORTED;
  }
  if (p->in_mode == VV_IN_POOL || p->in_mode == VV_IN_CUBE)
    return VV_ERR_UNSUPPORTED;
  hipStream_t st = (hipStream_t)stream;
  if (vv_wino_ring_ok(p)) return p->CinP == 16 ? launch_wino_ring<2>(p, st) : launch_wino_ring<4>(p, st);
  switch (p->H) {
    case 32: return launch_wino<32>(p, st);
    case 16: return launch_wino<16>(p, st);
    case 8: return launch_wino<8>(p, st);
    case 4: return launch_wino<4>(p, st);
  }
  return VV_ERR_UNSUPPORTED;
}

extern "C" int vv_pack_wino(const vv_pack_entry* table_dev, int32_t nentries, int32_t G, const float* params,
                            int64_t params_gstride, float* packed, int64_t packed_gstride, int32_t max_kn,
                            vv_stream stream) {
  if (!table_dev || !params || !packed || nentries <= 0) return VV_ERR_BAD_ARG;
  int bx = (max_kn + VV_WG - 1) / VV_WG;
  if (bx > 64) bx = 64;
  if (bx < 1) bx = 1;
  VV_LAUNCH(wino_pack_kernel, dim3(bx, nentries, G), dim3(VV_WG), 0, (hipStream_t)stream, table_dev, params, params_gstride,
            packed, packed_gstride);
  VV_CHECK_LAUNCH();
  return VV_OK;
}
```

Baseline: 28340.

## Fold BN-backward apply into dgrad and wgrad operand loads for selected layers

For selected conv layers, the separate BN-backward apply pass that wrote dz is dropped. A sums kernel now writes a 7-row per-channel table (a, b, mean, invstd, gamma*invstd, c1, c2). The Winograd dgrad conv and the wgrad kernel then recompute dz on the fly from dA and y while loading their operands. This removes one full elementwise read/write pass over the activation for each folded layer. In exchange both consumers read two tensors, the dgrad drops to the single-N-block variant, an extra LDS table and sync are added, and the BN math is done twice.

```diff
diff --git a/include/vecvad_hip.h b/include/vecvad_hip.h
--- a/include/vecvad_hip.h
+++ b/include/vecvad_hip.h
@@ -22,7 +22,8 @@
   VV_IN_ACT = 1,
   VV_IN_POOL = 2,
   VV_IN_CAT = 3,
-  VV_IN_CUBE = 4
+  VV_IN_CUBE = 4,
+  VV_IN_BNBWD = 5
 };
 
 enum vv_conv_kind {
@@ -93,6 +94,8 @@
   vv_view dy;
   float* partial;
   int64_t partial_gstride;
+  vv_view dy_z;
+  const float* dy_bn; int64_t dy_bn_gstride;
 } vv_wgrad_params;
 
 int vv_wgrad_mfma(const vv_wgrad_params* p, vv_stream stream);
@@ -161,6 +164,9 @@
 int vv_bn_bwd_nblk(int32_t B, int32_t H, int32_t W, int32_t C);
 int vv_bn_bwd_apply(const vv_bnbwd_params* p, const float* gamma, int64_t param_gstride, float* dgamma, float* dbeta,
                     int64_t grad_gstride, float* scratch , vv_stream stream);
+#define VV_BNBWD_TAB_ROWS 7
+int vv_bn_bwd_sums(const vv_bnbwd_params* p, const float* gamma, int64_t param_gstride, float* dgamma, float* dbeta,
+                   int64_t grad_gstride, float* table, int64_t table_gstride, vv_stream stream);
 
 typedef struct vv_outconv_params {
   int32_t G, B, HW, C;
diff --git a/vec_vad_amd/_lib.py b/vec_vad_amd/_lib.py
--- a/vec_vad_amd/_lib.py
+++ b/vec_vad_amd/_lib.py
@@ -8,7 +8,8 @@
 
 c_i32, c_i64, c_f32, c_f64, c_vp = C.c_int32, C.c_int64, C.c_float, C.c_double, C.c_void_p
 
-IN_PLAIN, IN_ACT, IN_POOL, IN_CAT, IN_CUBE = 0, 1, 2, 3, 4
+IN_PLAIN, IN_ACT, IN_POOL, IN_CAT, IN_CUBE, IN_BNBWD = 0, 1, 2, 3, 4, 5
+BNBWD_TAB_ROWS = 7
 CONV3, CONVT_FWD, CONVT_DGRAD = 0, 1, 2
 CONV_BF16 = 1
 CONV_SRC_BF16 = 2
@@ -51,7 +52,8 @@
                 ('Cin', c_i32), ('CinP', c_i32), ('Cout', c_i32), ('ksplit', c_i32),
                 ('src0', View), ('a', c_vp), ('b', c_vp), ('ab_gstride', c_i64),
                 ('src1', View), ('csplit', c_i32), ('pad0', c_i32), ('chmap', c_vp),
-                ('dy', View), ('partial', c_vp), ('partial_gstride', c_i64)]
+                ('dy', View), ('partial', c_vp), ('partial_gstride', c_i64),
+                ('dy_z', View), ('dy_bn', c_vp), ('dy_bn_gstride', c_i64)]
 
 
 class PackEntry(C.Structure):
@@ -122,6 +124,7 @@
     'vv_bn_bwd_reduce': (c_i32, [C.POINTER(BnBwdParams), c_vp]),
     'vv_bn_bwd_nblk': (c_i32, [c_i32, c_i32, c_i32, c_i32]),
     'vv_bn_bwd_apply': (c_i32, [C.POINTER(BnBwdParams), c_vp, c_i64, c_vp, c_vp, c_i64, c_vp, c_vp]),
+    'vv_bn_bwd_sums': (c_i32, [C.POINTER(BnBwdParams), c_vp, c_i64, c_vp, c_vp, c_i64, c_vp, c_i64, c_vp]),
     'vv_outconv_fwd': (c_i32, [C.POINTER(OutconvParams), c_vp]),
     'vv_outconv_bwd': (c_i32, [c_i32, c_i32, c_i32, c_i32, c_vp, c_vp, c_i64, c_vp, c_vp, c_i64, c_vp, c_i64,
                                c_vp, c_i64, c_vp, c_vp, c_vp, c_vp, c_i32, c_vp]),
diff --git a/vec_vad_amd/bank.py b/vec_vad_amd/bank.py
--- a/vec_vad_amd/bank.py
+++ b/vec_vad_amd/bank.py
@@ -787,6 +787,19 @@
                     fused_t[u] = sidx
         fused |= set(fused_t.values())
 
+        fold_env = os.environ.get('VV_FUSE_BN_APPLY', '1').lower()
+        fold_set = {int(t) for t in fold_env[4:].split(',') if t} if fold_env.startswith('set:') else \
+            (set() if fold_env in ('0', 'off') else {0, 2, 4})
+
+        def folded(l):
+            if l.idx not in fold_set or self.cflag or not self.wino or not self.wino_wgrad or l.idx == last.idx:
+                return False
+            if self.dz16 or self.da16 or self.y16 or l.H == 4 or l.cout > 256 or dA_for(l)[1] is not None:
+                return False
+            return l.idx == 0 or (l.H in (16, 8) and not self._w44(B, l, True))
+        fold = {l.idx for l in lay.convs if folded(l)}
+        ws.bntab = {i: f(Ga, L.BNBWD_TAB_ROWS * lay.convs[i].cout) for i in fold}
+
         def dgrad_flags(i):
             dz16 = bool(self.dz16 and len(wplan['c%d' % i]) > 2)
             return (self.cflag | ((L.CONV_ALLSRC_BF16 if self.y16 else L.CONV_SRC_BF16) if dz16 else 0) |
@@ -812,11 +825,20 @@
                                self._p(ws.ab[2, i]), self._p(ws.ab[3, i]), abg, dA, dpool, dpg, dzb.data_ptr(), dzb.stride(0),
                                ws.bnpart.data_ptr())
             P.keep.append(bp)
+            fl = i in fold
+            if fl:
+                reuse_wait = ()
             if not (from_outconv or from_dgrad):
                 P.add(lib.vv_bn_bwd_reduce, (C.byref(bp),), 'bn_bwd_reduce%d' % i, wait=reuse_wait)
-            P.add(lib.vv_bn_bwd_apply, (C.byref(bp), pbase + 4 * lay.p['c%d.g' % i][0], U, self._g('c%d.g' % i)[0],
-                                        self._g('c%d.beta' % i)[0], self._g('c%d.g' % i)[1], ws.bnscr.data_ptr()), 'bn_bwd_apply%d' % i,
-                  record='dy%d' % i, wait=reuse_wait if (from_outconv or from_dgrad) else ())
+            if fl:
+                tab = ws.bntab[i]
+                P.add(lib.vv_bn_bwd_sums, (C.byref(bp), pbase + 4 * lay.p['c%d.g' % i][0], U, self._g('c%d.g' % i)[0],
+                                           self._g('c%d.beta' % i)[0], self._g('c%d.g' % i)[1], tab.data_ptr(), tab.stride(0)),
+                      'bn_bwd_sum%d' % i, record='dy%d' % i)
+            else:
+                P.add(lib.vv_bn_bwd_apply, (C.byref(bp), pbase + 4 * lay.p['c%d.g' % i][0], U, self._g('c%d.g' % i)[0],
+                                            self._g('c%d.beta' % i)[0], self._g('c%d.g' % i)[1], ws.bnscr.data_ptr()), 'bn_bwd_apply%d' % i,
+                      record='dy%d' % i, wait=reuse_wait if (from_outconv or from_dgrad) else ())
             if i > 0:
                 Dl = ws.D[i]
                 w44 = self._w44(B, l, True)
@@ -826,6 +848,9 @@
                                   kbase + 4 * (lay.pkw44 if w44 else lay.pkw if self.wino else lay.pk)['c%d.d' % i][0], UP, None, 0,
                                   L.view(Dl, l.cin, 0, Dl.stride(0)),
                                   ws.dstats.data_ptr() if l.mode == L.IN_CAT else None)
+                if fl:
+                    cp.in_mode, cp.src0, cp.src1 = L.IN_BNBWD, dA, L.view(y, l.cout, 0, y.stride(0))
+                    cp.a, cp.ab_gstride = ws.bntab[i].data_ptr(), ws.bntab[i].stride(0)
                 if l.mode == L.IN_CAT:
                     v0, v1, osplit = dcat_views(l)
                     if osplit:
@@ -847,6 +872,9 @@
             wp = L.WgradParams(L.CONV3, mode, Ga, B, l.H, l.H, l.cin, l.cinp, l.cout, ks, s0, a, b, abg, s1, csplit,
                                wflag, chmap,
                                L.View(dzb.data_ptr(), dzb.stride(0), l.cout, 0), ws.wpart.data_ptr() + 4 * woff['c%d' % i], wpg)
+            if fl:
+                wp.dy, wp.dy_z = dA, L.view(y, l.cout, 0, y.stride(0))
+                wp.dy_bn, wp.dy_bn_gstride = ws.bntab[i].data_ptr(), ws.bntab[i].stride(0)
             P.keep.append(wp)
             P.add(lib.vv_wgrad_bf16 if kw else lib.vv_wgrad_mfma, (C.byref(wp),), 'wgrad%d' % i, stream=1, wait=('dy%d' % i,),
                   record='wdone%d' % i, pwait=('*main',))
diff --git a/vec_vad_amd/csrc/vv_common.h b/vec_vad_amd/csrc/vv_common.h
--- a/vec_vad_amd/csrc/vv_common.h
+++ b/vec_vad_amd/csrc/vv_common.h
@@ -58,6 +58,31 @@
   v.z = fmaxf(fmaf(a.z, v.z, b.z), 0.f);
   v.w = fmaxf(fmaf(a.w, v.w, b.w), 0.f);
   return v;
+}
+struct VVBnBwd4 { float4 a, b, m, i, gk, c1, c2; };
+__device__ __forceinline__ VVBnBwd4 vv_bnbwd_consts(const float* tab, const int C, const int c) {
+  VVBnBwd4 k;
+  k.a = *reinterpret_cast<const float4*>(tab + c);
+  k.b = *reinterpret_cast<const float4*>(tab + C + c);
+  k.m = *reinterpret_cast<const float4*>(tab + 2 * C + c);
+  k.i = *reinterpret_cast<const float4*>(tab + 3 * C + c);
+  k.gk = *reinterpret_cast<const float4*>(tab + 4 * C + c);
+  k.c1 = *reinterpret_cast<const float4*>(tab + 5 * C + c);
+  k.c2 = *reinterpret_cast<const float4*>(tab + 6 * C + c);
+  return k;
+}
+__device__ __forceinline__ float vv_bnbwd1(float d, const float y, const float a, const float b, const float m, const float i,
+                                           const float gk, const float c1, const float c2) {
+  const float z = fmaf(a, y, b);
+  d = z > 0.f ? d : 0.f;
+  const float xh = (y - m) * i;
+  return gk * (d - c1 - xh * c2);
+}
+__device__ __forceinline__ float4 vv_bnbwd4(const float4 d, const float4 y, const VVBnBwd4& k) {
+  return make_float4(vv_bnbwd1(d.x, y.x, k.a.x, k.b.x, k.m.x, k.i.x, k.gk.x, k.c1.x, k.c2.x),
+                     vv_bnbwd1(d.y, y.y, k.a.y, k.b.y, k.m.y, k.i.y, k.gk.y, k.c1.y, k.c2.y),
+                     vv_bnbwd1(d.z, y.z, k.a.z, k.b.z, k.m.z, k.i.z, k.gk.z, k.c1.z, k.c2.z),
+                     vv_bnbwd1(d.w, y.w, k.a.w, k.b.w, k.m.w, k.i.w, k.gk.w, k.c1.w, k.c2.w));
 }
 __device__ __forceinline__ float4 vv_max4(float4 p, float4 q) {
   p.x = fmaxf(p.x, q.x); p.y = fmaxf(p.y, q.y); p.z = fmaxf(p.z, q.z); p.w = fmaxf(p.w, q.w);
diff --git a/vec_vad_amd/csrc/vv_conv.hip b/vec_vad_amd/csrc/vv_conv.hip
--- a/vec_vad_amd/csrc/vv_conv.hip
+++ b/vec_vad_amd/csrc/vv_conv.hip
@@ -485,6 +485,7 @@
   if (!p || !p->src0.ptr || !p->w || !p->out.ptr) return VV_ERR_BAD_ARG;
   if (p->G <= 0 || p->B <= 0) return VV_ERR_BAD_ARG;
   if (p->Cout % 32) return VV_ERR_UNSUPPORTED;
+  if (p->in_mode == VV_IN_BNBWD) return VV_ERR_UNSUPPORTED;
   hipStream_t st = (hipStream_t)stream;
   const bool bf = (p->pad0 & VV_CONV_BF16) != 0;
   if (bf && p->CinP % 16) return VV_ERR_BAD_ARG;
diff --git a/vec_vad_amd/csrc/vv_elem.hip b/vec_vad_amd/csrc/vv_elem.hip
--- a/vec_vad_amd/csrc/vv_elem.hip
+++ b/vec_vad_amd/csrc/vv_elem.hip
@@ -142,12 +142,13 @@
   const float4 a4 = *reinterpret_cast<const float4*>(p.a + abo), b4 = *reinterpret_cast<const float4*>(p.b + abo);
   const float4 m4 = *reinterpret_cast<const float4*>(p.mean + abo), i4 = *reinterpret_cast<const float4*>(p.invstd + abo);
   float4 s1 = make_float4(0, 0, 0, 0), s2 = make_float4(0, 0, 0, 0);
-  float4 gk = make_float4(0, 0, 0, 0), c1 = gk, c2 = gk;
+  VVBnBwd4 kc;
   if constexpr (PASS == 1) {
     const float4 gm = *reinterpret_cast<const float4*>(gamma + (int64_t)g * param_gstride + c);
-    gk = make_float4(gm.x * i4.x, gm.y * i4.y, gm.z * i4.z, gm.w * i4.w);
-    c1 = *reinterpret_cast<const float4*>(scratch + (int64_t)g * 2 * C + c);
-    c2 = *reinterpret_cast<const float4*>(scratch + (int64_t)g * 2 * C + C + c);
+    kc.a = a4; kc.b = b4; kc.m = m4; kc.i = i4;
+    kc.gk = make_float4(gm.x * i4.x, gm.y * i4.y, gm.z * i4.z, gm.w * i4.w);
+    kc.c1 = *reinterpret_cast<const float4*>(scratch + (int64_t)g * 2 * C + c);
+    kc.c2 = *reinterpret_cast<const float4*>(scratch + (int64_t)g * 2 * C + C + c);
   }
 
   const bool y16 = (p.flags & VV_BNBWD_Y_BF16) != 0;
@@ -156,16 +157,15 @@
     return *reinterpret_cast<const float4*>(y + pix * C + c);
   };
   auto one = [&](const int64_t pix, float4 d, const float4 yv) {
-    float4 z;
-    z.x = fmaf(a4.x, yv.x, b4.x); z.y = fmaf(a4.y, yv.y, b4.y); z.z = fmaf(a4.z, yv.z, b4.z); z.w = fmaf(a4.w, yv.w, b4.w);
-    d.x = z.x > 0.f ? d.x : 0.f; d.y = z.y > 0.f ? d.y : 0.f; d.z = z.z > 0.f ? d.z : 0.f; d.w = z.w > 0.f ? d.w : 0.f;
-    const float4 xh = make_float4((yv.x - m4.x) * i4.x, (yv.y - m4.y) * i4.y, (yv.z - m4.z) * i4.z, (yv.w - m4.w) * i4.w);
     if constexpr (PASS == 0) {
+      float4 z;
+      z.x = fmaf(a4.x, yv.x, b4.x); z.y = fmaf(a4.y, yv.y, b4.y); z.z = fmaf(a4.z, yv.z, b4.z); z.w = fmaf(a4.w, yv.w, b4.w);
+      d.x = z.x > 0.f ? d.x : 0.f; d.y = z.y > 0.f ? d.y : 0.f; d.z = z.z > 0.f ? d.z : 0.f; d.w = z.w > 0.f ? d.w : 0.f;
+      const float4 xh = make_float4((yv.x - m4.x) * i4.x, (yv.y - m4.y) * i4.y, (yv.z - m4.z) * i4.z, (yv.w - m4.w) * i4.w);
       s1.x += d.x; s1.y += d.y; s1.z += d.z; s1.w += d.w;
       s2.x = fmaf(d.x, xh.x, s2.x); s2.y = fmaf(d.y, xh.y, s2.y); s2.z = fmaf(d.z, xh.z, s2.z); s2.w = fmaf(d.w, xh.w, s2.w);
     } else {
-      d.x = gk.x * (d.x - c1.x - xh.x * c2.x); d.y = gk.y * (d.y - c1.y - xh.y * c2.y);
-      d.z = gk.z * (d.z - c1.z - xh.z * c2.z); d.w = gk.w * (d.w - c1.w - xh.w * c2.w);
+      d = vv_bnbwd4(d, yv, kc);
       if (p.flags & VV_BNBWD_DZ_BF16) *reinterpret_cast<uint2*>(reinterpret_cast<unsigned short*>(dz) + pix * C + c) = vv_pack_bf16x4(d);
       else *reinterpret_cast<float4*>(dz + pix * C + c) = d;
     }
@@ -348,7 +348,8 @@
 __global__ void __launch_bounds__(32 * VV_NP)
 bn_bwd_sum_kernel(const int C, const int nblk, const double M, const float* __restrict__ partial,
                   float* __restrict__ dgamma, float* __restrict__ dbeta, const int64_t grad_gstride,
-                  float* __restrict__ scratch) {
+                  float* __restrict__ scratch, const vv_bnbwd_params tp, const float* __restrict__ gamma,
+                  const int64_t param_gstride, float* __restrict__ tab, const int64_t tab_gstride) {
   __shared__ double sh[2][VV_NP][32];
   const int g = blockIdx.y;
   const int cl = threadIdx.x & 31, part = threadIdx.x >> 5;
@@ -367,8 +368,21 @@
   for (int k = 0; k < VV_NP; ++k) { s1 += sh[0][k][cl]; s2 += sh[1][k][cl]; }
   dbeta[(int64_t)g * grad_gstride + c] = (float)s1;
   dgamma[(int64_t)g * grad_gstride + c] = (float)s2;
-  scratch[(int64_t)g * 2 * C + c] = (float)(s1 / M);
-  scratch[(int64_t)g * 2 * C + C + c] = (float)(s2 / M);
+  if (!tab) {
+    scratch[(int64_t)g * 2 * C + c] = (float)(s1 / M);
+    scratch[(int64_t)g * 2 * C + C + c] = (float)(s2 / M);
+    return;
+  }
+  float* t = tab + (int64_t)g * tab_gstride + c;
+  const int64_t o = (int64_t)g * tp.ab_gstride + c;
+  const float iv = tp.invstd[o];
+  t[0] = tp.a[o];
+  t[C] = tp.b[o];
+  t[2 * C] = tp.mean[o];
+  t[3 * C] = iv;
+  t[4 * C] = gamma[(int64_t)g * param_gstride + c] * iv;
+  t[5 * C] = (float)(s1 / M);
+  t[6 * C] = (float)(s2 / M);
 }
 
 template <int CC>
@@ -1284,19 +1298,37 @@
   return VV_OK;
 }
 
+static inline int bn_partial_rows(const vv_bnbwd_params* p) {
+  return (p->flags & VV_BNBWD_PARTIALS_PER_CUBE) ? p->B
+         : (p->flags & VV_BNBWD_PARTIALS_PER_TILE) ? vv_wino_ntiles(p->B, p->H)
+         : (p->flags & VV_BNBWD_PARTIALS_PER_TILE44) ? vv_wino44_ntiles(p->B, p->H)
+         : (p->flags & VV_BNBWD_PARTIALS_PER_CTILE) ? vv_conv_ntiles(p->B, p->H, p->W)
+         : (p->flags & VV_BNBWD_PARTIALS_PER_TTILE) ? vv_convt_dgrad_ntiles(p->B, p->H, p->W, 0) : bn_nblk_of(p);
+}
+
+extern "C" int vv_bn_bwd_sums(const vv_bnbwd_params* p, const float* gamma, int64_t param_gstride, float* dgamma, float* dbeta,
+                              int64_t grad_gstride, float* table, int64_t table_gstride, vv_stream stream) {
+  if (!p || !p->partial || !p->a || !p->b || !p->mean || !p->invstd || !gamma || !dgamma || !dbeta || !table) return VV_ERR_BAD_ARG;
+  if (p->dpool || (p->flags & (VV_BNBWD_DZ_BF16 | VV_BNBWD_DA_BF16 | VV_BNBWD_Y_BF16))) return VV_ERR_UNSUPPORTED;
+  if (table_gstride < (int64_t)VV_BNBWD_TAB_ROWS * p->C) return VV_ERR_BAD_ARG;
+  const int nblk = bn_partial_rows(p);
+  if (nblk <= 0) return VV_ERR_BAD_ARG;
+  const int64_t M = (int64_t)p->B * p->H * p->W;
+  VV_LAUNCH(bn_bwd_sum_kernel, dim3((p->C + 31) / 32, p->G), dim3(32 * VV_NP), 0, (hipStream_t)stream, p->C, nblk, (double)M,
+            p->partial, dgamma, dbeta, grad_gstride, nullptr, *p, gamma, param_gstride, table, table_gstride);
+  VV_CHECK_LAUNCH();
+  return VV_OK;
+}
+
 extern "C" int vv_bn_bwd_apply(const vv_bnbwd_params* p, const float* gamma, int64_t param_gstride, float* dgamma,
                                float* dbeta, int64_t grad_gstride, float* scratch, vv_stream stream) {
   if (!p || !p->y || !p->dA.ptr || !p->dz || !p->partial || !gamma || !dgamma || !dbeta || !scratch) return VV_ERR_BAD_ARG;
-  const int nblk = (p->flags & VV_BNBWD_PARTIALS_PER_CUBE) ? p->B
-                   : (p->flags & VV_BNBWD_PARTIALS_PER_TILE) ? vv_wino_ntiles(p->B, p->H)
-                   : (p->flags & VV_BNBWD_PARTIALS_PER_TILE44) ? vv_wino44_ntiles(p->B, p->H)
-                   : (p->flags & VV_BNBWD_PARTIALS_PER_CTILE) ? vv_conv_ntiles(p->B, p->H, p->W)
-                   : (p->flags & VV_BNBWD_PARTIALS_PER_TTILE) ? vv_convt_dgrad_ntiles(p->B, p->H, p->W, 0) : bn_nblk_of(p);
+  const int nblk = bn_partial_rows(p);
   if (nblk <= 0) return VV_ERR_BAD_ARG;
   const int nblk_apply = bn_nblk_of(p);
   const int64_t M = (int64_t)p->B * p->H * p->W;
   VV_LAUNCH(bn_bwd_sum_kernel, dim3((p->C + 31) / 32, p->G), dim3(32 * VV_NP), 0, (hipStream_t)stream, p->C, nblk, (double)M,
-            p->partial, dgamma, dbeta, grad_gstride, scratch);
+            p->partial, dgamma, dbeta, grad_gstride, scratch, *p, nullptr, 0, nullptr, 0);
   VV_CHECK_LAUNCH();
   if (bn_all16(p)) {
     if (p->dpool)
diff --git a/vec_vad_amd/csrc/vv_wgrad.hip b/vec_vad_amd/csrc/vv_wgrad.hip
--- a/vec_vad_amd/csrc/vv_wgrad.hip
+++ b/vec_vad_amd/csrc/vv_wgrad.hip
@@ -196,7 +196,7 @@
   for (int j = 0; j < 9; ++j) out[tid + j * VV_WG] = l4[tid + j * VV_WG];
 }
 
-template <int TH, int TW, int NI, int UH, int UNI>
+template <int TH, int TW, int NI, int UH, int UNI, bool BNB>
 __global__ void __launch_bounds__(256, 3)
 wgrad_wino_kernel(const vv_wgrad_params p, const int NT, const int NCI, const int NCO, const int total, const int nper) {
   constexpr int NTH = 256, W_ = TW;
@@ -245,6 +245,17 @@
   const float* baseB = p.dy.ptr + (int64_t)g * p.dy.gstride + p.dy.coff;
   const int csB = p.dy.cstride;
 
+  const float* baseZ = BNB ? p.dy_z.ptr + (int64_t)g * p.dy_z.gstride + p.dy_z.coff : nullptr;
+  const int csZ = p.dy_z.cstride;
+  __shared__ float bnk[BNB ? VV_BNBWD_TAB_ROWS * 32 : 1];
+  if constexpr (BNB) {
+    if (tid < VV_BNBWD_TAB_ROWS * 32)
+      bnk[tid] = p.dy_bn[(int64_t)g * p.dy_bn_gstride + (tid >> 5) * p.Cout + cot * 32 + (tid & 31)];
+  }
+  unsigned voffZ[BNB ? NPB : 1];
+  float4 rz[BNB ? NPB : 1];
+  __amdgpu_buffer_rsrc_t rsZ;
+
   unsigned voffA[NPA], voffB[NPB];
   int slotA[NPA];
   unsigned topm = 0, botm = 0;
@@ -268,6 +279,7 @@
     const int px = (tid + k * NTH) >> 3;
     const int im = px / (UH * W_), rem = px % (UH * W_);
     voffB[k] = (unsigned)((im * H * W_ + rem) * csB + cB) * 4u;
+    if constexpr (BNB) voffZ[k] = (unsigned)((im * H * W_ + rem) * csZ + cB) * 4u;
   }
 
   int pt_n = ks, u_n = 0;
@@ -285,6 +297,9 @@
     const int64_t ob = ((int64_t)(img0 * H + uy0) * W_) * csB;
     rsA = __builtin_amdgcn_make_buffer_rsrc(const_cast<float*>(baseA + oa), 0, 0x7FFFFFFF, 0x00020000);
     rsB = __builtin_amdgcn_make_buffer_rsrc(const_cast<float*>(baseB + ob), 0, 0x7FFFFFFF, 0x00020000);
+    if constexpr (BNB)
+      rsZ = __builtin_amdgcn_make_buffer_rsrc(const_cast<float*>(baseZ + ((int64_t)(img0 * H + uy0) * W_) * csZ), 0, 0x7FFFFFFF,
+                                              0x00020000);
     const bool img_ok = live && img0 < p.B;
     kill = img_ok ? 0u : 0xFFFFFFFFu;
     if (ROWDYN) {
@@ -314,6 +329,10 @@
     } else {
       const v4f v = __builtin_amdgcn_raw_buffer_load_b128(rsB, liveB[k - NPA] ? voffB[k - NPA] : OOB, 0, 0);
       r[k] = make_float4(v.x, v.y, v.z, v.w);
+      if constexpr (BNB) {
+        const v4f z = __builtin_amdgcn_raw_buffer_load_b128(rsZ, liveB[k - NPA] ? voffZ[k - NPA] : OOB, 0, 0);
+        rz[k - NPA] = make_float4(z.x, z.y, z.z, z.w);
+      }
     }
   };
   auto commit_piece = [&](auto K, float* buf) {
@@ -325,7 +344,11 @@
         *reinterpret_cast<float4*>(buf + slotA[k]) = v;
       }
     } else {
-      *reinterpret_cast<float4*>(buf + ASZ + ((tid + (k - NPA) * NTH) >> 3) * 32 + q8 * 4) = r[k];
+      float4 v = r[k];
+      if constexpr (BNB) {
+        if (liveB[k - NPA]) v = vv_bnbwd4(v, rz[k - NPA], vv_bnbwd_consts(bnk, 32, q8 * 4));
+      }
+      *reinterpret_cast<float4*>(buf + ASZ + ((tid + (k - NPA) * NTH) >> 3) * 32 + q8 * 4) = v;
     }
   };
 
@@ -366,6 +389,7 @@
 #pragma unroll
     for (int i = 0; i < 16; ++i) acc[n][i] = 0.f;
 
+  if constexpr (BNB) __syncthreads();
   begin_unit();
   vv_static_for<0, NP>([&](auto K) { load_piece(K); });
   vv_static_for<0, NP>([&](auto K) { commit_piece(K, lds); });
@@ -512,16 +536,24 @@
   return false;
 }
 
-template <int TH, int TW, int NI, int UH, int UNI>
-int launch_ww(const vv_wgrad_params* p, hipStream_t st) {
+template <int TH, int TW, int NI, int UH, int UNI, bool BNB>
+int launch_ww_(const vv_wgrad_params* p, hipStream_t st) {
   if (p->W != TW) return VV_ERR_UNSUPPORTED;
   const int NT = ((p->B + NI - 1) / NI) * (p->H / TH) * (p->W / TW);
   const int NCI = (p->CinP + 31) / 32, NCO = p->Cout / 32;
   const int total = p->G * NCI * NCO * p->ksplit;
   const int nper = (total + 7) / 8;
-  VV_LAUNCH((wgrad_wino_kernel<TH, TW, NI, UH, UNI>), dim3(nper * 8), dim3(256), 0, st, *p, NT, NCI, NCO, total, nper);
+  VV_LAUNCH((wgrad_wino_kernel<TH, TW, NI, UH, UNI, BNB>), dim3(nper * 8), dim3(256), 0, st, *p, NT, NCI, NCO, total, nper);
   VV_CHECK_LAUNCH();
   return VV_OK;
+}
+
+template <int TH, int TW, int NI, int UH, int UNI>
+int launch_ww(const vv_wgrad_params* p, hipStream_t st) {
+  if constexpr (TW == 4) {
+    if (p->dy_bn) return VV_ERR_UNSUPPORTED;
+  } else if (p->dy_bn) return launch_ww_<TH, TW, NI, UH, UNI, true>(p, st);
+  return launch_ww_<TH, TW, NI, UH, UNI, false>(p, st);
 }
 
 template <int TH, int TW, int NI, int KIND>
@@ -549,6 +581,11 @@
   if (p->Cout % 32 || p->ksplit < 1) return VV_ERR_BAD_ARG;
   if (p->kind == VV_CONV3 && (p->in_mode == VV_IN_POOL || p->in_mode == VV_IN_CUBE))
     return VV_ERR_UNSUPPORTED;
+  if (p->in_mode == VV_IN_BNBWD) return VV_ERR_UNSUPPORTED;
+  if (p->dy_bn) {
+    if (p->kind != VV_CONV3 || !(p->pad0 & 256) || !p->dy_z.ptr) return VV_ERR_UNSUPPORTED;
+    if ((int64_t)p->B * p->H * p->W * p->dy_z.cstride * 4 >= (1ll << 31)) return VV_ERR_UNSUPPORTED;
+  }
   hipStream_t st = (hipStream_t)stream;
   if (p->kind == VV_CONV3 && (p->pad0 & 256)) {
     switch (p->H) {
diff --git a/vec_vad_amd/csrc/vv_wgrad_bf16.hip b/vec_vad_amd/csrc/vv_wgrad_bf16.hip
--- a/vec_vad_amd/csrc/vv_wgrad_bf16.hip
+++ b/vec_vad_amd/csrc/vv_wgrad_bf16.hip
@@ -811,6 +811,7 @@
   if (!p || !p->src0.ptr || !p->dy.ptr || !p->partial) return VV_ERR_BAD_ARG;
   if (p->Cout % 32 || p->ksplit < 1) return VV_ERR_BAD_ARG;
   if (p->in_mode == VV_IN_POOL || p->in_mode == VV_IN_CUBE) return VV_ERR_UNSUPPORTED;
+  if (p->dy_bn || p->in_mode == VV_IN_BNBWD) return VV_ERR_UNSUPPORTED;
   hipStream_t st = (hipStream_t)stream;
   if ((p->pad0 & VV_WGRAD_DY_BF16) && p->dy.coff % 2) return VV_ERR_BAD_ARG;
   if ((p->pad0 & VV_WGRAD_X_BF16) && !(p->pad0 & VV_WGRAD_DY_BF16)) return VV_ERR_UNSUPPORTED;
diff --git a/vec_vad_amd/csrc/vv_wino.hip b/vec_vad_amd/csrc/vv_wino.hip
--- a/vec_vad_amd/csrc/vv_wino.hip
+++ b/vec_vad_amd/csrc/vv_wino.hip
@@ -30,7 +30,7 @@
   static constexpr int HH = 2 * TROWS + 2, HW = H_ + 2;
 };
 
-template <int H_, int NB>
+template <int H_, int NB, bool BNB>
 __global__ void __launch_bounds__(WN, NB == 2 ? 2 : 3)
 wino_conv_kernel(const vv_conv_params p, const int NT, const int NN, const int total, const int nper) {
   using G_ = WGeo<H_>;
@@ -99,8 +99,33 @@
       voff[k] = ((valid >> k) & 1u) ? (unsigned)((tile + pixv[k]) * cs + q4) * 4u : 0x80000000u;
     cur_second = second ? 1 : 0;
   };
+  float4 rz[BNB ? NIT : 1];
+  unsigned zoff[BNB ? NIT : 1];
+  __shared__ float bnt[BNB ? VV_BNBWD_TAB_ROWS * 256 : 1];
+  int cur_c = 0;
+  __amdgpu_buffer_rsrc_t rsZ;
+  if constexpr (BNB) {
+    rsZ = __builtin_amdgcn_make_buffer_rsrc(const_cast<float*>(s.p1 + s.co1), 0, 0x7FFFFFFF, 0x00020000);
+#pragma unroll
+    for (int k = 0; k < NIT; ++k)
+      zoff[k] = ((valid >> k) & 1u) ? (unsigned)((tile + pixv[k]) * s.cs1 + q4) * 4u : 0x80000000u;
+    for (int i = tid; i < VV_BNBWD_TAB_ROWS * CinP; i += WN) bnt[i] = s.a[i];
+    __syncthreads();
+  }
   auto issue = [&](const int c0) {
     const int c = c0 + q4;
+    if constexpr (BNB) {
+      if (cur_second != 0) set_source(false);
+      cur_c = c;
+#pragma unroll
+      for (int k = 0; k < NIT; ++k) {
+        const v4f v = __builtin_amdgcn_raw_buffer_load_b128(rs, voff[k], c0 * 4, 0);
+        r[k] = make_float4(v.x, v.y, v.z, v.w);
+        const v4f z = __builtin_amdgcn_raw_buffer_load_b128(rsZ, zoff[k], c0 * 4, 0);
+        rz[k] = make_float4(z.x, z.y, z.z, z.w);
+      }
+      return;
+    }
     act = (s.mode == VV_IN_ACT) || (s.mode == VV_IN_CAT && c < s.csplit);
     if (act) {
       sa = *reinterpret_cast<const float4*>(s.a + c);
@@ -115,11 +140,15 @@
     }
   };
   auto commit = [&]() {
+    VVBnBwd4 kc;
+    if constexpr (BNB) kc = vv_bnbwd_consts(bnt, CinP, cur_c);
 #pragma unroll
     for (int k = 0; k < NIT; ++k)
       if (NITEMS % WN == 0 || k < NIT - 1 || slot[k] >= 0) {
         float4 v = r[k];
-        if (act && ((valid >> k) & 1u)) v = vv_act4(v, sa, sb);
+        if constexpr (BNB) {
+          if ((valid >> k) & 1u) v = vv_bnbwd4(v, rz[k], kc);
+        } else if (act && ((valid >> k) & 1u)) v = vv_act4(v, sa, sb);
         lds4[slot[k]] = v;
       }
   };
@@ -702,7 +731,7 @@
   using G_ = WGeo<H_>;
   const int NT = ((p->B + G_::NI - 1) / G_::NI) * G_::PARTS;
   static const bool nb1 = [] { const char* e = getenv("VV_WINO_NB"); return e && e[0] == '1'; }();
-  bool two = !nb1 && p->Cout % 64 == 0;
+  bool two = !nb1 && p->Cout % 64 == 0 && p->in_mode != VV_IN_BNBWD;
   if (two) {
     const int64_t wgs = (int64_t)p->G * (p->Cout / 64) * NT;
     const int64_t rounds = (wgs + 511) / 512;
@@ -711,10 +740,15 @@
   const int NN = p->Cout / (two ? 64 : 32);
   const int total = p->G * NN * NT;
   const int nper = (total + 7) / 8;
+  const bool bnb = p->in_mode == VV_IN_BNBWD;
   if (two)
-    VV_LAUNCH((wino_conv_kernel<H_, 2>), dim3(nper * 8), dim3(WN), 0, st, *p, NT, NN, total, nper);
+    VV_LAUNCH((wino_conv_kernel<H_, 2, false>), dim3(nper * 8), dim3(WN), 0, st, *p, NT, NN, total, nper);
+  else if constexpr (H_ != 4) {
+    if (bnb) VV_LAUNCH((wino_conv_kernel<H_, 1, true>), dim3(nper * 8), dim3(WN), 0, st, *p, NT, NN, total, nper);
+    else VV_LAUNCH((wino_conv_kernel<H_, 1, false>), dim3(nper * 8), dim3(WN), 0, st, *p, NT, NN, total, nper);
+  }
   else
-    VV_LAUNCH((wino_conv_kernel<H_, 1>), dim3(nper * 8), dim3(WN), 0, st, *p, NT, NN, total, nper);
+    VV_LAUNCH((wino_conv_kernel<H_, 1, false>), dim3(nper * 8), dim3(WN), 0, st, *p, NT, NN, total, nper);
   VV_CHECK_LAUNCH();
   return VV_OK;
 }
@@ -744,6 +778,11 @@
   }
   if (p->in_mode == VV_IN_POOL || p->in_mode == VV_IN_CUBE)
     return VV_ERR_UNSUPPORTED;
+  if (p->in_mode == VV_IN_BNBWD) {
+    if (!p->src1.ptr || !p->a || p->Cin != p->CinP || (p->pad0 & (VV_CONV_BF16 | VV_CONV_RELU))) return VV_ERR_BAD_ARG;
+    if (p->H == 4 || p->CinP > 256) return VV_ERR_UNSUPPORTED;
+    if ((int64_t)p->B * p->H * p->W * p->src1.cstride * 4 >= (1ll << 31)) return VV_ERR_UNSUPPORTED;
+  }
   hipStream_t st = (hipStream_t)stream;
   if (vv_wino_ring_ok(p)) return p->CinP == 16 ? launch_wino_ring<2>(p, st) : launch_wino_ring<4>(p, st);
   switch (p->H) {
```

Result: faster. 28840 (median of 6 runs) (+1.8%).
